# josegarciav/PINNs-RL-PDE

Measured on AMD Instinct MI355X. Metric: collocation-points/sec (residual+grad) + final residual L2, Burgers 1D, higher is better.
Workload: dtype f32

## Files before the change

include/pinn_jet.h:

```cpp
#ifndef PINN_JET_H
#define PINN_JET_H

#include <stddef.h>
#include <stdint.h>

#ifdef __cplusplus
extern "C" {
#endif

#define PINN_ABI_VERSION 2
#define PINN_MAX_LINEAR 24
#define PINN_MAX_STREAMS 7

#define PINN_FLAG_LAYER_NORM 1
#define PINN_FLAG_DETERMINISTIC 2
#define PINN_FLAG_LAYER_MAJOR 4
#define PINN_FLAG_WIDE_TILE32 8
#define PINN_FLAG_PLAIN_STREAMS 16
#define PINN_FLAG_SPACE_AXIS(a) ((a) << 8)
#define PINN_FLAG_SPACE_AXIS_MASK 0x300
#define PINN_FLAG_SPACE_DIRECTION(d0, d1, d2) \
  (((((d0) < 0 ? 2 : (d0)) & 3) << 10) | ((((d1) < 0 ? 2 : (d1)) & 3) << 12) | ((((d2) < 0 ? 2 : (d2)) & 3) << 14))
#define PINN_FLAG_SPACE_DIRECTION_MASK 0xFC00

typedef enum PinnStatus {
  PINN_OK = 0,
  PINN_ERR_BAD_DESC = -1,
  PINN_ERR_UNSUPPORTED = -2,
  PINN_ERR_MISALIGNED = -3,
  PINN_ERR_WORKSPACE = -4,
  PINN_ERR_HIP = -5,
  PINN_ERR_BAD_ORDER = -6
} PinnStatus;

typedef enum PinnArch {
  PINN_ARCH_FEEDFORWARD = 0,
  PINN_ARCH_FOURIER = 1,
  PINN_ARCH_SIREN = 2,
  PINN_ARCH_RESNET = 3,
  PINN_ARCH_ATTENTION = 4,
  PINN_ARCH_AUTOENCODER = 5
} PinnArch;

typedef enum PinnAct {
  PINN_ACT_TANH = 0,
  PINN_ACT_SIN = 1,
  PINN_ACT_GELU = 2,
  PINN_ACT_SIGMOID = 3,
  PINN_ACT_RELU = 4,
  PINN_ACT_LEAKY_RELU = 5,
  PINN_ACT_IDENTITY = 6
} PinnAct;

typedef enum PinnPde {
  PINN_PDE_BURGERS = 0,
  PINN_PDE_HEAT = 1,
  PINN_PDE_ALLEN_CAHN = 2,
  PINN_PDE_KDV = 3,
  PINN_PDE_CAHN_HILLIARD = 4,
  PINN_PDE_WAVE = 5,
  PINN_PDE_CONVECTION = 6,
  PINN_PDE_BLACK_SCHOLES = 7,
  PINN_PDE_PENDULUM = 8,
  PINN_PDE_HEAT_LAPLACIAN = 9
} PinnPde;

typedef enum PinnLoss { PINN_LOSS_MSE = 0, PINN_LOSS_MAE = 1, PINN_LOSS_HUBER = 2 } PinnLoss;

typedef struct PinnNetDesc {
  int32_t arch;
  int32_t activation;
  int32_t input_dim;
  int32_t num_linear;
  int32_t widths[PINN_MAX_LINEAR];
  int32_t mapping_size;
  float act_param;
  float ln_eps;
  int32_t num_blocks;
  int32_t flags;
} PinnNetDesc;

typedef struct PinnPdeDesc {
  int32_t kind;
  int32_t dimension;
  int32_t loss;
  float coef[4];
  float huber_delta;
} PinnPdeDesc;

int pinn_abi_version(void);
const char* pinn_last_error(void);

const char* pinn_build_info(void);

int pinn_num_tensors(const PinnNetDesc* net);

int pinn_pde_streams(const PinnPdeDesc* pde, int32_t* time_order, int32_t* space_order);

size_t pinn_workspace_bytes(const PinnNetDesc* net, int64_t N, int32_t time_order, int32_t space_order, int32_t backward);

typedef struct PinnKernelInfo {
  int32_t engine;
  int32_t time_order, space_order, act_family, backward;
  int32_t hmax, na0;
  int32_t grid;
  int32_t flush;
  int32_t default_mfma_form;
} PinnKernelInfo;
int pinn_kernel_for(const PinnNetDesc* net, int64_t N, int32_t time_order, int32_t space_order, int32_t backward,
                    PinnKernelInfo* out);
int pinn_kernel_name(const PinnNetDesc* net, int64_t N, int32_t time_order, int32_t space_order, int32_t backward,
                     char* buf, size_t len);

#define PINN_LM_MAX_PLAN 41
typedef struct PinnLmNodePlan {
  int32_t rows, depth;
  int32_t width;
  int32_t has_ln, has_skip, has_add;
  int32_t act_family;
  int32_t src_kind;
  int32_t fwd_fused;
  int32_t fwd_nch, fwd_rt, fwd_gy, fwd_aux;
  int32_t fwd_ew_kind;
  int32_t fwd_fpt;
  int32_t bwd_fused;
  int32_t bwd_nch, bwd_rt, bwd_gy, bwd_aux;
  int32_t bwd_ew_kind;
  int32_t bwd_fpt;
  int32_t head_fpt;
} PinnLmNodePlan;
int pinn_lm_plan(const PinnNetDesc* net, int64_t N, int32_t time_order, int32_t space_order, int32_t backward,
                 PinnLmNodePlan* out, int32_t max_records);

int pinn_unit_tail_plan(int64_t N, int32_t grid, int64_t* rounds, int32_t* groups, int64_t* first_tail_point);


int pinn_jet_forward(const PinnNetDesc* net, const float* const* weights, int32_t num_tensors, const float* x,
                     const float* t, int64_t N, int32_t time_order, int32_t space_order, float* const* jets_out,
                     void* workspace, size_t ws_bytes, void* stream);

int pinn_jet_backward(const PinnNetDesc* net, const float* const* weights, int32_t num_tensors, const float* x,
                      const float* t, int64_t N, int32_t time_order, int32_t space_order,
                      const float* const* jet_cotangents, float* const* weight_grads, void* workspace, size_t ws_bytes,
                      void* stream);

int pinn_jet_backward_inputs(const PinnNetDesc* net, const float* const* weights, int32_t num_tensors, const float* x,
                             const float* t, int64_t N, int32_t time_order, int32_t space_order,
                             const float* const* jet_cotangents, float* const* weight_grads,
                             float* x_grad, float* t_grad, void* workspace, size_t ws_bytes, void* stream);

int pinn_residual_forward(const PinnNetDesc* net, const float* const* weights, int32_t num_tensors,
                          const PinnPdeDesc* pde, const float* x, const float* t, int64_t N, float* residual_out,
                          float* loss_sum_out, void* workspace, size_t ws_bytes, void* stream);

int pinn_residual_loss_grad(const PinnNetDesc* net, const float* const* weights, int32_t num_tensors,
                            const PinnPdeDesc* pde, const float* x, const float* t, int64_t N, float grad_scale,
                            float* residual_out, float* loss_sum_out, float* const* weight_grads, void* workspace,
                            size_t ws_bytes, void* stream);

int pinn_residual_loss_grad_coef(const PinnNetDesc* net, const float* const* weights, int32_t num_tensors,
                                 const PinnPdeDesc* pde, const float* x, const float* t, int64_t N, float grad_scale,
                                 float* residual_out, float* loss_sum_out, float* const* weight_grads, float* coef_grads,
                                 void* workspace, size_t ws_bytes, void* stream);

int pinn_residual_loss_grad_inverse(const PinnNetDesc* net, const float* const* weights, int32_t num_tensors,
                                    const PinnPdeDesc* pde, const float* coef_values, const float* x, const float* t,
                                    int64_t N, float grad_scale, float* residual_out, float* loss_sum_out,
                                    float* const* weight_grads, float* coef_grads, void* workspace, size_t ws_bytes,
                                    void* stream);
size_t pinn_inverse_workspace_bytes(const PinnNetDesc* net, const PinnPdeDesc* pde, int64_t N);
int pinn_inverse_kernel_name(const PinnNetDesc* net, const PinnPdeDesc* pde, int64_t N, char* buf, size_t len);

int pinn_residual_backward(const PinnNetDesc* net, const float* const* weights, int32_t num_tensors,
                           const PinnPdeDesc* pde, const float* x, const float* t, int64_t N,
                           const float* residual_cotangent, float* const* weight_grads, void* workspace,
                           size_t ws_bytes, void* stream);

#define PINN_MAX_POINT_TERMS 8

int pinn_point_losses(const float* u, int32_t n_total, int32_t n_terms, const int32_t* lo, const int32_t* hi,
                      const float* const* targets, const float* weights, int32_t loss, float huber_delta,
                      float* term_losses, float* cotangent, const float* residual_sum, float residual_scale,
                      float residual_weight, int32_t n_boundary_terms, float* summary4, void* stream);

int pinn_jet_losses(const float* jets, int32_t n_streams, int32_t n_total, int32_t n_terms, const int32_t* lo, const int32_t* hi,
                    const int32_t* stream_of, const int32_t* pair_offset, const float* const* targets, const float* weights,
                    int32_t loss, float huber_delta, float* term_losses, float* cotangent, const float* residual_sum,
                    float residual_scale, float residual_weight, int32_t n_boundary_terms, float* summary4, void* stream);

#define PINN_FD_SCRATCH_DOUBLES 128
int pinn_fd_stencil_points(const float* x, const float* t, int64_t N, double eps, double x_lo, double x_hi, float* x3, float* t3,
                           void* stream);
int pinn_fd_smoothness(const float* u3, int64_t N, double eps, float weight, float* loss_out, float* cotangent3, float* summary4,
                       double* scratch, void* stream);

#define PINN_CAUSAL_MAX_BINS 64
#define PINN_CAUSAL_SCRATCH_DOUBLES (64 * 2 * PINN_CAUSAL_MAX_BINS)
int pinn_causal_weights(const float* residual, const float* t, int64_t N, int32_t n_bins, double t_lo, double t_hi,
                        const float* eps_dev, int32_t loss, float huber_delta, float grad_scale, float* cotangent,
                        float* loss_sum_out, float* plain_sum_out, float* bin_losses, float* bin_weights, double* scratch,
                        void* stream);

#define PINN_TERM_MAX_TERMS 16
#define PINN_TERM_MAX_FACTORS 4
#define PINN_TERM_SCRATCH_DOUBLES (64 * (1 + PINN_TERM_MAX_TERMS))

typedef enum PinnTermFactor {
  PINN_TERM_U = 0,
  PINN_TERM_UT = 1,
  PINN_TERM_UTT = 2,
  PINN_TERM_UX = 3,
  PINN_TERM_UXX = 4,
  PINN_TERM_UXXX = 5,
  PINN_TERM_UXXXX = 6,
  PINN_TERM_X = 7,
  PINN_TERM_T = 8,
  PINN_TERM_SIN_U = 9,
  PINN_TERM_COS_U = 10
} PinnTermFactor;

typedef struct PinnTermPdeTerm {
  int32_t n_factors;
  int32_t factor[PINN_TERM_MAX_FACTORS];
} PinnTermPdeTerm;

typedef struct PinnTermPde {
  int32_t time_order, space_order;
  int32_t n_terms;
  int32_t loss;
  float huber_delta;
  PinnTermPdeTerm terms[PINN_TERM_MAX_TERMS];
} PinnTermPde;

int pinn_term_residual(const PinnTermPde* pde, const float* coef_values, const float* jets, const float* x, const float* t,
                       int64_t N, float grad_scale, const float* residual_cotangent, float* residual_out, float* loss_sum_out,
                       float* jet_cotangents, float* coef_grads, double* scratch, void* stream);

#define PINN_TERM_UY 11
#define PINN_TERM_UYY 12
#define PINN_TERM_UZ 13
#define PINN_TERM_UZZ 14
#define PINN_TERM_Y 15
#define PINN_TERM_Z 16

typedef struct PinnTermPdeAxes {
  int32_t dimension;
  int32_t time_order;
  int32_t space_order[3];
  int32_t n_terms;
  int32_t loss;
  float huber_delta;
  PinnTermPdeTerm terms[PINN_TERM_MAX_TERMS];
} PinnTermPdeAxes;

int pinn_term_residual_axes(const PinnTermPdeAxes* pde, const float* coef_values, const float* const* jets, const float* x,
                            const float* t, int64_t N, float grad_scale, const float* residual_cotangent, float* residual_out,
                            float* loss_sum_out, float* const* jet_cotangents, float* coef_grads, double* scratch, void* stream);

#define PINN_TERM_UYYY 17
#define PINN_TERM_UYYYY 18
#define PINN_TERM_UZZZ 19
#define PINN_TERM_UZZZZ 20
#define PINN_TERM_UXY 21
#define PINN_TERM_UXZ 22
#define PINN_TERM_UYZ 23
#define PINN_TERM_UXXYY 24
#define PINN_TERM_UXXZZ 25
#define PINN_TERM_UYYZZ 26
#define PINN_TERM_MIXED_BLOCKS 9

typedef struct PinnTermPdeMixed {
  int32_t dimension;
  int32_t time_order;
  int32_t space_order[3];
  int32_t pair_order[3];
  int32_t n_terms;
  int32_t loss;
  float huber_delta;
  PinnTermPdeTerm terms[PINN_TERM_MAX_TERMS];
} PinnTermPdeMixed;

int pinn_term_residual_mixed(const PinnTermPdeMixed* pde, const float* coef_values, const float* const* jets, const float* x,
                             const float* t, int64_t N, float grad_scale, const float* residual_cotangent, float* residual_out,
                             float* loss_sum_out, float* const* jet_cotangents, float* coef_grads, double* scratch, void* stream);

#define PINN_SYSTEM_MAX_FIELDS 4
#define PINN_SYSTEM_MAX_EQUATIONS 4
#define PINN_SYSTEM_MAX_TERMS 32
#define PINN_SYSTEM_SCRATCH_DOUBLES (64 * (4 + 32))
#define PINN_SYSTEM_FACTOR(field, code) ((field) * 32 + (code))

typedef struct PinnTermPdeSystem {
  int32_t dimension;
  int32_t n_fields;
  int32_t n_equations;
  int32_t time_order[PINN_SYSTEM_MAX_FIELDS];
  int32_t space_order[PINN_SYSTEM_MAX_FIELDS][3];
  int32_t n_terms;
  int32_t equation_of[PINN_SYSTEM_MAX_TERMS];
  float eq_weight[PINN_SYSTEM_MAX_EQUATIONS];
  int32_t loss;
  float huber_delta;
  PinnTermPdeTerm terms[PINN_SYSTEM_MAX_TERMS];
} PinnTermPdeSystem;

int pinn_term_residual_system(const PinnTermPdeSystem* pde, const float* coef_values, const float* const* jets, const float* x,
                              const float* t, int64_t N, float grad_scale, const float* residual_cotangent, float* residual_out,
                              float* loss_sum_out, float* eq_loss_sums, float* const* jet_cotangents, float* coef_grads,
                              double* scratch, void* stream);

int pinn_adam_clip_step(float* params, const float* grads, float* exp_avg, float* exp_avg_sq, int64_t n, const float* lr,
                        float beta1, float beta2, float eps, float weight_decay, float max_norm, float* step,
                        float* scratch64, float* grad_norm_out, void* stream);

#define PINN_ADAPTIVE_RBW 0
#define PINN_ADAPTIVE_LRW 1
#define PINN_ADAPTIVE_SCRATCH_FLOATS 1296
int pinn_adaptive_adam_step(float* params, const float* comp_grads, int64_t ld, int32_t n_components,
                            const float* const* comp_losses, const float* loss_scales, int32_t strategy, double alpha,
                            double aw_eps, const float* initial_weights, float* state16, float* weights4_out, float* summary4,
                            float* exp_avg, float* exp_avg_sq, int64_t n, const float* lr, float beta1, float beta2, float eps,
                            float weight_decay, float max_norm, float* step, float* scratch, float* grad_norm_out,
                            float* grad_out, void* stream);

#define PINN_LBFGS_MAX_HISTORY 64
#define PINN_LBFGS_RECORD_DOUBLES 72
#define PINN_LBFGS_REC_LOSS 0
#define PINN_LBFGS_REC_GTD 1
#define PINN_LBFGS_REC_GMAX 2
#define PINN_LBFGS_REC_GSUM 3
#define PINN_LBFGS_REC_ACCEPTED 4
#define PINN_LBFGS_REC_COUNT 5
#define PINN_LBFGS_REC_ITER 6
#define PINN_LBFGS_REC_HDIAG 7
#define PINN_LBFGS_REC_DMAX 8
size_t pinn_lbfgs_state_bytes(int32_t history_size);
size_t pinn_lbfgs_scratch_bytes(int32_t history_size);
int pinn_lbfgs_direction(const float* grad, float* prev_grad, float* direction, float* ring, int64_t ld, int64_t n,
                         int32_t history_size, double t_prev, double* state, double* scratch, double* record, void* stream);
int pinn_lbfgs_eval_stats(const float* grad, const float* direction, int64_t n, const float* loss, double* scratch,
                          double* record, void* stream);

#ifdef __cplusplus
}
#endif
#endif
```

pinns-rl-pde_amd/_lib.py:

```python

from __future__ import annotations

import ctypes
import os
import subprocess
import threading

_HERE = os.path.dirname(os.path.abspath(__file__))
LIB_PATH = os.environ.get("PINN_LIB") or os.path.join(_HERE, "libpinnjet.so")
CSRC = os.path.join(_HERE, "csrc")

PINN_ABI_VERSION = 2
PINN_MAX_LINEAR = 24
PINN_MAX_STREAMS = 7
PINN_FLAG_LAYER_NORM = 1
PINN_FLAG_DETERMINISTIC = 2
PINN_FLAG_LAYER_MAJOR = 4
PINN_FLAG_WIDE_TILE32 = 8
PINN_FLAG_PLAIN_STREAMS = 16
PINN_FLAG_SPACE_AXIS_MASK = 0x300


def PINN_FLAG_SPACE_AXIS(axis: int) -> int:
    return (int(axis) << 8) & PINN_FLAG_SPACE_AXIS_MASK


PINN_FLAG_SPACE_DIRECTION_MASK = 0xFC00


def PINN_FLAG_SPACE_DIRECTION(d0: int = 0, d1: int = 0, d2: int = 0) -> int:
    bits = 0
    for a, d in enumerate((d0, d1, d2)):
        if d not in (-1, 0, 1):
            raise ValueError(f"direction entry {d!r}: -1, 0 or +1")
        bits |= (2 if d < 0 else int(d)) << (10 + 2 * a)
    return bits


ARCH = {"feedforward": 0, "fourier": 1, "siren": 2, "resnet": 3, "attention": 4, "autoencoder": 5}
ACT = {"tanh": 0, "sin": 1, "gelu": 2, "sigmoid": 3, "relu": 4, "leaky_relu": 5, "identity": 6}
PDE = {
    "burgers": 0, "heat": 1, "allen_cahn": 2, "kdv": 3, "cahn_hilliard": 4, "wave": 5, "convection": 6,
    "black_scholes": 7, "pendulum": 8, "heat_laplacian": 9,
}
LOSS = {"mse": 0, "mae": 1, "huber": 2}
ADAPTIVE = {"rbw": 0, "lrw": 1}
PINN_ADAPTIVE_SCRATCH_FLOATS = 1296
PINN_FD_SCRATCH_DOUBLES = 128
PINN_LBFGS_MAX_HISTORY = 64
PINN_LBFGS_RECORD_DOUBLES = 72
PINN_TERM_MAX_TERMS = 16
PINN_TERM_MAX_FACTORS = 4
PINN_TERM_SCRATCH_DOUBLES = 64 * (1 + PINN_TERM_MAX_TERMS)
PINN_CAUSAL_MAX_BINS = 64
PINN_CAUSAL_SCRATCH_DOUBLES = 64 * 2 * PINN_CAUSAL_MAX_BINS
TERM_FACTOR = {"u": 0, "u_t": 1, "u_tt": 2, "u_x": 3, "u_xx": 4, "u_xxx": 5, "u_xxxx": 6, "x": 7, "t": 8, "sin(u)": 9, "cos(u)": 10}
TERM_FACTOR_ND = dict(TERM_FACTOR, **{"u_y": 11, "u_yy": 12, "u_z": 13, "u_zz": 14, "y": 15, "z": 16})
TERM_FACTOR_MIXED = dict(TERM_FACTOR_ND, **{"u_yyy": 17, "u_yyyy": 18, "u_zzz": 19, "u_zzzz": 20, "u_xy": 21, "u_xz": 22, "u_yz": 23,
                                            "u_xxyy": 24, "u_xxzz": 25, "u_yyzz": 26})
PINN_TERM_MIXED_BLOCKS = 9
PINN_SYSTEM_MAX_FIELDS = 4
PINN_SYSTEM_MAX_EQUATIONS = 4
PINN_SYSTEM_MAX_TERMS = 32
PINN_SYSTEM_SCRATCH_DOUBLES = 64 * (4 + 32)


def PINN_SYSTEM_FACTOR(field: int, code: int) -> int:
    return int(field) * 32 + int(code)


LBFGS_REC = {"loss": 0, "gtd": 1, "gmax": 2, "gsum": 3, "accepted": 4, "count": 5, "n_iter": 6, "h_diag": 7, "dmax": 8}

EXPORTS = (
    "pinn_abi_version", "pinn_last_error", "pinn_build_info", "pinn_num_tensors", "pinn_pde_streams",
    "pinn_workspace_bytes", "pinn_jet_forward", "pinn_jet_backward", "pinn_residual_forward", "pinn_residual_backward",
    "pinn_residual_loss_grad", "pinn_residual_loss_grad_coef", "pinn_point_losses", "pinn_jet_losses", "pinn_adam_clip_step",
    "pinn_jet_backward_inputs", "pinn_kernel_for", "pinn_kernel_name", "pinn_residual_loss_grad_inverse",
    "pinn_inverse_workspace_bytes", "pinn_inverse_kernel_name", "pinn_adaptive_adam_step", "pinn_lbfgs_state_bytes",
    "pinn_lbfgs_scratch_bytes", "pinn_lbfgs_direction", "pinn_lbfgs_eval_stats", "pinn_fd_stencil_points", "pinn_fd_smoothness",
    "pinn_unit_tail_plan", "pinn_term_residual", "pinn_causal_weights", "pinn_term_residual_axes",
    "pinn_term_residual_mixed", "pinn_lm_plan", "pinn_term_residual_system",
)


class PinnNetDesc(ctypes.Structure):
    _fields_ = [
        ("arch", ctypes.c_int32), ("activation", ctypes.c_int32), ("input_dim", ctypes.c_int32),
        ("num_linear", ctypes.c_int32), ("widths", ctypes.c_int32 * PINN_MAX_LINEAR),
        ("mapping_size", ctypes.c_int32), ("act_param", ctypes.c_float), ("ln_eps", ctypes.c_float),
        ("num_blocks", ctypes.c_int32), ("flags", ctypes.c_int32),
    ]


class PinnPdeDesc(ctypes.Structure):
    _fields_ = [
        ("kind", ctypes.c_int32), ("dimension", ctypes.c_int32), ("loss", ctypes.c_int32),
        ("coef", ctypes.c_float * 4), ("huber_delta", ctypes.c_float),
    ]


class PinnTermPdeTerm(ctypes.Structure):
    _fields_ = [("n_factors", ctypes.c_int32), ("factor", ctypes.c_int32 * PINN_TERM_MAX_FACTORS)]


class PinnTermPde(ctypes.Structure):
    _fields_ = [
        ("time_order", ctypes.c_int32), ("space_order", ctypes.c_int32), ("n_terms", ctypes.c_int32), ("loss", ctypes.c_int32),
        ("huber_delta", ctypes.c_float), ("terms", PinnTermPdeTerm * PINN_TERM_MAX_TERMS),
    ]


class PinnTermPdeAxes(ctypes.Structure):
    _fields_ = [
        ("dimension", ctypes.c_int32), ("time_order", ctypes.c_int32), ("space_order", ctypes.c_int32 * 3),
        ("n_terms", ctypes.c_int32), ("loss", ctypes.c_int32), ("huber_delta", ctypes.c_float),
        ("terms", PinnTermPdeTerm * PINN_TERM_MAX_TERMS),
    ]


class PinnTermPdeMixed(ctypes.Structure):
    _fields_ = [
        ("dimension", ctypes.c_int32), ("time_order", ctypes.c_int32), ("space_order", ctypes.c_int32 * 3),
        ("pair_order", ctypes.c_int32 * 3), ("n_terms", ctypes.c_int32), ("loss", ctypes.c_int32),
        ("huber_delta", ctypes.c_float), ("terms", PinnTermPdeTerm * PINN_TERM_MAX_TERMS),
    ]


class PinnTermPdeSystem(ctypes.Structure):
    _fields_ = [
        ("dimension", ctypes.c_int32), ("n_fields", ctypes.c_int32), ("n_equations", ctypes.c_int32),
        ("time_order", ctypes.c_int32 * PINN_SYSTEM_MAX_FIELDS), ("space_order", (ctypes.c_int32 * 3) * PINN_SYSTEM_MAX_FIELDS),
        ("n_terms", ctypes.c_int32), ("equation_of", ctypes.c_int32 * PINN_SYSTEM_MAX_TERMS),
        ("eq_weight", ctypes.c_float * PINN_SYSTEM_MAX_EQUATIONS), ("loss", ctypes.c_int32), ("huber_delta", ctypes.c_float),
        ("terms", PinnTermPdeTerm * PINN_SYSTEM_MAX_TERMS),
    ]


class PinnKernelInfo(ctypes.Structure):
    _fields_ = [
        ("engine", ctypes.c_int32), ("time_order", ctypes.c_int32), ("space_order", ctypes.c_int32),
        ("act_family", ctypes.c_int32), ("backward", ctypes.c_int32), ("hmax", ctypes.c_int32), ("na0", ctypes.c_int32),
        ("grid", ctypes.c_int32), ("flush", ctypes.c_int32), ("default_mfma_form", ctypes.c_int32),
    ]


PINN_LM_MAX_PLAN = 41


class PinnLmNodePlan(ctypes.Structure):
    _fields_ = [(f, ctypes.c_int32) for f in (
        "rows", "depth", "width", "has_ln", "has_skip", "has_add", "act_family", "src_kind",
        "fwd_fused", "fwd_nch", "fwd_rt", "fwd_gy", "fwd_aux", "fwd_ew_kind", "fwd_fpt",
        "bwd_fused", "bwd_nch", "bwd_rt", "bwd_gy", "bwd_aux", "bwd_ew_kind", "bwd_fpt", "head_fpt")]


ENGINE_LAYER_MAJOR, ENGINE_TILE_MAJOR = 0, 1
FLUSH = {0: "direct", 1: "store", 2: "two_level", 3: "deterministic"}


class JetLibraryError(RuntimeError):
    """The HIP library is missing, stale, or returned an error code."""


_lib = None
_lock = threading.Lock()


def build(verbose: bool = False) -> str:
    cmd = ["make", "-C", CSRC, "-j", str(min(8, os.cpu_count() or 1))]
    res = subprocess.run(cmd, stdout=subprocess.PIPE, stderr=subprocess.STDOUT, text=True)
    if verbose or res.returncode:
        print(res.stdout)
    if res.returncode:
        raise JetLibraryError(f"building libpinnjet.so failed (exit {res.returncode})")
    return LIB_PATH


def load():
    global _lib
    if _lib is not None:
        return _lib
    with _lock:
        if _lib is not None:
            return _lib
        if not os.path.exists(LIB_PATH):
            raise JetLibraryError(
                f"{LIB_PATH} not found: the HIP extension is not built (run `python -c 'import __graft_entry__ as g; "
                "g.build()'` or `make -C pinns-rl-pde_amd/csrc`).  There is no CPU fallback."
            )
        import torch

        lib = ctypes.CDLL(LIB_PATH)
        vp, i32, i64, f32 = ctypes.c_void_p, ctypes.c_int32, ctypes.c_int64, ctypes.c_float
        P = ctypes.POINTER
        lib.pinn_abi_version.restype = ctypes.c_int
        lib.pinn_abi_version.argtypes = []
        lib.pinn_last_error.restype = ctypes.c_char_p
        lib.pinn_last_error.argtypes = []
        lib.pinn_build_info.restype = ctypes.c_char_p
        lib.pinn_build_info.argtypes = []
        lib.pinn_num_tensors.restype = ctypes.c_int
        lib.pinn_num_tensors.argtypes = [P(PinnNetDesc)]
        lib.pinn_pde_streams.restype = ctypes.c_int
        lib.pinn_pde_streams.argtypes = [P(PinnPdeDesc), P(i32), P(i32)]
        lib.pinn_workspace_bytes.restype = ctypes.c_size_t
        lib.pinn_workspace_bytes.argtypes = [P(PinnNetDesc), i64, i32, i32, i32]
        sz = ctypes.c_size_t
        lib.pinn_kernel_for.restype = ctypes.c_int
        lib.pinn_kernel_for.argtypes = [P(PinnNetDesc), i64, i32, i32, i32, P(PinnKernelInfo)]
        lib.pinn_kernel_name.restype = ctypes.c_int
        lib.pinn_kernel_name.argtypes = [P(PinnNetDesc), i64, i32, i32, i32, ctypes.c_char_p, sz]
        lib.pinn_lm_plan.restype = ctypes.c_int
        lib.pinn_lm_plan.argtypes = [P(PinnNetDesc), i64, i32, i32, i32, P(PinnLmNodePlan), i32]
        lib.pinn_jet_forward.restype = ctypes.c_int
        lib.pinn_jet_forward.argtypes = [P(PinnNetDesc), P(vp), i32, vp, vp, i64, i32, i32, P(vp), vp, sz, vp]
        lib.pinn_jet_backward.restype = ctypes.c_int
        lib.pinn_jet_backward.argtypes = [P(PinnNetDesc), P(vp), i32, vp, vp, i64, i32, i32, P(vp), P(vp), vp, sz, vp]
        lib.pinn_jet_backward_inputs.restype = ctypes.c_int
        lib.pinn_jet_backward_inputs.argtypes = [P(PinnNetDesc), P(vp), i32, vp, vp, i64, i32, i32, P(vp), P(vp), vp, vp, vp,
                                                 sz, vp]
        lib.pinn_residual_forward.restype = ctypes.c_int
        lib.pinn_residual_forward.argtypes = [P(PinnNetDesc), P(vp), i32, P(PinnPdeDesc), vp, vp, i64, vp, vp, vp, sz, vp]
        lib.pinn_residual_backward.restype = ctypes.c_int
        lib.pinn_residual_backward.argtypes = [P(PinnNetDesc), P(vp), i32, P(PinnPdeDesc), vp, vp, i64, vp, P(vp), vp, sz,
                                               vp]
        lib.pinn_residual_loss_grad.restype = ctypes.c_int
        lib.pinn_residual_loss_grad.argtypes = [P(PinnNetDesc), P(vp), i32, P(PinnPdeDesc), vp, vp, i64, f32, vp, vp,
                                                P(vp), vp, sz, vp]
        lib.pinn_residual_loss_grad_coef.restype = ctypes.c_int
        lib.pinn_residual_loss_grad_coef.argtypes = [P(PinnNetDesc), P(vp), i32, P(PinnPdeDesc), vp, vp, i64, f32, vp, vp,
                                                     P(vp), vp, vp, sz, vp]
        lib.pinn_residual_loss_grad_inverse.restype = ctypes.c_int
        lib.pinn_residual_loss_grad_inverse.argtypes = [P(PinnNetDesc), P(vp), i32, P(PinnPdeDesc), vp, vp, vp, i64, f32, vp, vp,
                                                        P(vp), vp, vp, sz, vp]
        lib.pinn_inverse_workspace_bytes.restype = ctypes.c_size_t
        lib.pinn_inverse_workspace_bytes.argtypes = [P(PinnNetDesc), P(PinnPdeDesc), i64]
        lib.pinn_inverse_kernel_name.restype = ctypes.c_int
        lib.pinn_inverse_kernel_name.argtypes = [P(PinnNetDesc), P(PinnPdeDesc), i64, ctypes.c_char_p, sz]
        lib.pinn_point_losses.restype = ctypes.c_int
        lib.pinn_point_losses.argtypes = [vp, i32, i32, P(i32), P(i32), P(vp), P(f32), i32, f32, vp, vp, vp, f32, f32, i32, vp, vp]
        lib.pinn_jet_losses.restype = ctypes.c_int
        lib.pinn_jet_losses.argtypes = [vp, i32, i32, i32, P(i32), P(i32), P(i32), P(i32), P(vp), P(f32), i32, f32, vp, vp, vp, f32, f32,
                                        i32, vp, vp]
        lib.pinn_adam_clip_step.restype = ctypes.c_int
        lib.pinn_adam_clip_step.argtypes = [vp, vp, vp, vp, i64, vp, f32, f32, f32, f32, f32, vp, vp, vp, vp]
        f64 = ctypes.c_double
        lib.pinn_adaptive_adam_step.restype = ctypes.c_int
        lib.pinn_adaptive_adam_step.argtypes = [vp, vp, i64, i32, P(vp), P(f32), i32, f64, f64, P(f32), vp, vp, vp, vp, vp, i64, vp,
                                                f32, f32, f32, f32, f32, vp, vp, vp, vp, vp]
        lib.pinn_lbfgs_state_bytes.restype = ctypes.c_size_t
        lib.pinn_lbfgs_state_bytes.argtypes = [i32]
        lib.pinn_lbfgs_scratch_bytes.restype = ctypes.c_size_t
        lib.pinn_lbfgs_scratch_bytes.argtypes = [i32]
        lib.pinn_lbfgs_direction.restype = ctypes.c_int
        lib.pinn_lbfgs_direction.argtypes = [vp, vp, vp, vp, i64, i64, i32, f64, vp, vp, vp, vp]
        lib.pinn_lbfgs_eval_stats.restype = ctypes.c_int
        lib.pinn_lbfgs_eval_stats.argtypes = [vp, vp, i64, vp, vp, vp, vp]
        lib.pinn_fd_stencil_points.restype = ctypes.c_int
        lib.pinn_fd_stencil_points.argtypes = [vp, vp, i64, f64, f64, f64, vp, vp, vp]
        lib.pinn_fd_smoothness.restype = ctypes.c_int
        lib.pinn_fd_smoothness.argtypes = [vp, i64, f64, f32, vp, vp, vp, vp, vp]
        lib.pinn_unit_tail_plan.restype = ctypes.c_int
        lib.pinn_unit_tail_plan.argtypes = [i64, i32, P(i64), P(i32), P(i64)]
        lib.pinn_term_residual.restype = ctypes.c_int
        lib.pinn_term_residual.argtypes = [P(PinnTermPde), vp, vp, vp, vp, i64, f32, vp, vp, vp, vp, vp, vp, vp]
        lib.pinn_term_residual_axes.restype = ctypes.c_int
        lib.pinn_term_residual_axes.argtypes = [P(PinnTermPdeAxes), vp, P(vp), vp, vp, i64, f32, vp, vp, vp, P(vp), vp, vp, vp]
        lib.pinn_term_residual_mixed.restype = ctypes.c_int
        lib.pinn_term_residual_mixed.argtypes = [P(PinnTermPdeMixed), vp, P(vp), vp, vp, i64, f32, vp, vp, vp, P(vp), vp, vp, vp]
        lib.pinn_term_residual_system.restype = ctypes.c_int
        lib.pinn_term_residual_system.argtypes = [P(PinnTermPdeSystem), vp, P(vp), vp, vp, i64, f32, vp, vp, vp, vp, P(vp), vp, vp, vp]
        lib.pinn_causal_weights.restype = ctypes.c_int
        lib.pinn_causal_weights.argtypes = [vp, vp, i64, i32, f64, f64, vp, i32, f32, f32, vp, vp, vp, vp, vp, vp, vp]
        if lib.pinn_abi_version() != PINN_ABI_VERSION:
            raise JetLibraryError(f"libpinnjet.so ABI {lib.pinn_abi_version()} != expected {PINN_ABI_VERSION}: rebuild")
        _lib = lib
    return _lib


def build_info() -> str:
    return load().pinn_build_info().decode("utf-8", "replace")


def kernel_for(prog, N: int, nt: int, nx: int, backward: int) -> dict:
    info = PinnKernelInfo()
    check(load().pinn_kernel_for(ctypes.byref(prog.desc), int(N), int(nt), int(nx), int(backward), ctypes.byref(info)))
    out = {f: getattr(info, f) for f, _ in PinnKernelInfo._fields_}
    out["engine"] = "tile_major" if info.engine == ENGINE_TILE_MAJOR else "layer_major"
    out["flush"] = FLUSH.get(info.flush)
    out["default_mfma_form"] = bool(info.default_mfma_form)
    return out


def lm_plan(prog, N: int, nt: int, nx: int, backward: int) -> list:
    recs = (PinnLmNodePlan * PINN_LM_MAX_PLAN)()
    n = load().pinn_lm_plan(ctypes.byref(prog.desc), int(N), int(nt), int(nx), int(backward), recs, PINN_LM_MAX_PLAN)
    if n < 0:
        check(n)
    return [{f: getattr(recs[m], f) for f, _ in PinnLmNodePlan._fields_} for m in range(n + 1)]


def kernel_name(prog, N: int, nt: int, nx: int, backward: int) -> str:
    buf = ctypes.create_string_buffer(64)
    check(load().pinn_kernel_name(ctypes.byref(prog.desc), int(N), int(nt), int(nx), int(backward), buf, len(buf)))
    return buf.value.decode("ascii")


def u16_tail_plan(N: int, grid: int) -> tuple:
    r, g, f = ctypes.c_int64(), ctypes.c_int32(), ctypes.c_int64()
    check(load().pinn_unit_tail_plan(int(N), int(grid), ctypes.byref(r), ctypes.byref(g), ctypes.byref(f)))
    return r.value, g.value, f.value


def check(rc: int) -> None:
    if rc != 0:
        msg = load().pinn_last_error().decode("utf-8", "replace")
        if rc == -6:
            raise ValueError(msg)
        if rc == -2:
            raise NotImplementedError(f"pinn_jet: {msg}")
        raise JetLibraryError(f"pinn_jet error {rc}: {msg}")
```

pinns-rl-pde_amd/csrc/jet_kernel_u16.h:

```cpp
#pragma once
#include "jet_kernel_wide.h"

namespace pinn {

#define U16_BARRIER(idx)     \
  do {                       \
    PINN_STAMP(idx);         \
    __syncthreads();         \
    PINN_STAMP(ST_BARRIER);  \
  } while (0)

constexpr int kU = 16;
constexpr int kUP = 132;
constexpr int kUThreads = 512;
constexpr int kUWaves = 8;
constexpr int kUH = 128;
constexpr int kUImgS = kU * kUP;

__device__ __forceinline__ f32x4 mfma16(float a, float b, f32x4 c) {
  return __builtin_amdgcn_mfma_f32_16x16x4f32(a, b, c, 0, 0, 0);
}

__device__ __forceinline__ int u16_opaque(int v) {
  asm volatile("" : "+v"(v));
  return v;
}

template <int NT, int NX>
__device__ __forceinline__ void u16_enc_preact(const float* ep, int din, const float* xin, int j, int n, float* z) {
  constexpr int K = 1 + NT + NX;
#pragma unroll
  for (int s = 0; s < K; ++s) z[s] = 0.0f;
  float v = ep[kMaxDin * kUH + j];
  float wt = 0.0f;
#pragma unroll
  for (int c = 0; c < kMaxDin; ++c) {
    const float w = ep[c * kUH + j];
    v = fmaf(xin[c * kU + n], w, v);
    wt = c == din - 1 ? w : wt;
  }
  z[0] = v;
  if constexpr (NT >= 1) z[1] = wt;
  if constexpr (NX >= 1) z[1 + NT] = ep[j];
}

template <int ACT, int NT, int NX, bool MRG = false>
__device__ __forceinline__ void u16_encode(const NetDev& net, const float* ep, const float* xin, float* dst, int tid, float cc = 0.0f) {
  constexpr int K = 1 + NT + NX;
  const int n = tid & 15;
  const int din = net.din;
  float* row = dst + n * kUP;
  if (net.enc == ENC_FOURIER) {
    const int M = net.enc_out >> 1;
#pragma unroll 1
    for (int m = tid >> 4; m < M; m += kUThreads / kU) {
      float z[K], ys[K], yc[K];
      u16_enc_preact<NT, NX>(ep, din, xin, m, n, z);
      float sn, cs;
      fast_sincosf(z[0], &sn, &cs);
      const float fs[6] = {sn, cs, -sn, -cs, sn, cs};
      const float fc[6] = {cs, -sn, -cs, sn, cs, -sn};
      ys[0] = sn;
      yc[0] = cs;
      if constexpr (MRG) {
        merged_fwd(fs, cc, z, ys);
        merged_fwd(fc, cc, z, yc);
      } else {
        dir_fwd<NT>(fs, z + 1, ys + 1);
        dir_fwd<NX>(fs, z + 1 + NT, ys + 1 + NT);
        dir_fwd<NT>(fc, z + 1, yc + 1);
        dir_fwd<NX>(fc, z + 1 + NT, yc + 1 + NT);
      }
#pragma unroll
      for (int s = 0; s < K; ++s) {
        row[s * kUImgS + m] = ys[s];
        row[s * kUImgS + M + m] = yc[s];
      }
    }
  } else {
    const int H = net.enc_out;
#pragma unroll 1
    for (int f = tid >> 4; f < H; f += kUThreads / kU) {
      float z[K], y[K];
      u16_enc_preact<NT, NX>(ep, din, xin, f, n, z);
      if constexpr (MRG) act_fwd_merged<ACT>(net.enc_param, cc, z, y);
      else act_fwd<ACT, NT, NX>(net.enc_param, z, y);
#pragma unroll
      for (int s = 0; s < K; ++s) row[s * kUImgS + f] = y[s];
    }
  }
}

__device__ __forceinline__ unsigned u16_rows_off(int row0, int ld, int c, int g) {
  return static_cast<unsigned>((row0 + c) * ld + 4 * g) * 4u;
}
__device__ __forceinline__ unsigned u16_cols_off(int col0, int ld, int c, int g) {
  return static_cast<unsigned>(4 * g * ld + col0 + c) * 4u;
}
template <bool COLS>
__device__ __forceinline__ f32x4 u16_wload(const float* W, int ld, unsigned off, int b) {
  if constexpr (COLS) {
    f32x4 v;
#pragma unroll
    for (int m = 0; m < 4; ++m) v[m] = *reinterpret_cast<const float*>(reinterpret_cast<const char*>(W + (long long)(16 * b + m) * ld) + off);
    return v;
  } else {
    return *reinterpret_cast<const f32x4*>(reinterpret_cast<const char*>(W + 16 * b) + off);
  }
}

template <int K, int NB, bool COLS>
__device__ __forceinline__ void u16_gemm_n(f32x4 (&acc)[K], const float* W, int ld, unsigned off, f32x4 w0, f32x4 w1, const float* xl) {
  f32x4 wq[3];
  wq[0] = w0;
  wq[1] = w1;
  f32x4 bc[K], bn[K];
#pragma unroll
  for (int s = 0; s < K; ++s) bc[s] = *reinterpret_cast<const f32x4*>(xl + s * kUImgS);
#pragma unroll
  for (int b = 0; b < NB; ++b) {
    if (b + 2 < NB) wq[(b + 2) % 3] = u16_wload<COLS>(W, ld, off, b + 2);
    if (b + 1 < NB) {
#pragma unroll
      for (int s = 0; s < K; ++s) bn[s] = *reinterpret_cast<const f32x4*>(xl + s * kUImgS + 16 * (b + 1));
    }
    __builtin_amdgcn_sched_barrier(0);
#pragma unroll
    for (int m = 0; m < 4; ++m)
#pragma unroll
      for (int s = 0; s < K; ++s) acc[s] = mfma16(wq[b % 3][m], bc[s][m], acc[s]);
    __builtin_amdgcn_sched_barrier(0);
    if (b + 1 < NB) {
#pragma unroll
      for (int s = 0; s < K; ++s) bc[s] = bn[s];
    }
  }
}

template <int K, bool COLS>
__device__ __forceinline__ void u16_gemm(f32x4 (&acc)[K], const float* W, int ld, unsigned off, f32x4 w0, f32x4 w1, int nb, const float* xl) {
  switch (nb) {
    case 8: u16_gemm_n<K, 8, COLS>(acc, W, ld, off, w0, w1, xl); return;
    case 4: u16_gemm_n<K, 4, COLS>(acc, W, ld, off, w0, w1, xl); return;
    default: break;
  }
#pragma unroll 1
  for (int b = 0; b < nb; ++b) {
    const f32x4 w = b == 0 ? w0 : b == 1 ? w1 : u16_wload<COLS>(W, ld, off, b);
#pragma unroll
    for (int m = 0; m < 4; ++m)
#pragma unroll
      for (int s = 0; s < K; ++s) acc[s] = mfma16(w[m], xl[s * kUImgS + 16 * b + m], acc[s]);
  }
}

template <int K, int NA, int OFF, int NPT>
__device__ __forceinline__ void u16_outer_n(f32x4 (&pt)[NPT], const float* zl, const float* al) {
  float zc, zn, ac[NA], an[NA];
  zc = zl[0];
#pragma unroll
  for (int t = 0; t < NA; ++t) ac[t] = al[16 * t];
#pragma unroll
  for (int st = 0; st < 4 * K; ++st) {
    if (st + 1 < 4 * K) {
      const int s = (st + 1) >> 2, m = (st + 1) & 3;
      zn = zl[s * kUImgS + m * kUP];
#pragma unroll
      for (int t = 0; t < NA; ++t) an[t] = al[s * kUImgS + m * kUP + 16 * t];
    }
    __builtin_amdgcn_sched_barrier(0);
#pragma unroll
    for (int t = 0; t < NA; ++t) pt[OFF + t] = mfma16(zc, ac[t], pt[OFF + t]);
    __builtin_amdgcn_sched_barrier(0);
    if (st + 1 < 4 * K) {
      zc = zn;
#pragma unroll
      for (int t = 0; t < NA; ++t) ac[t] = an[t];
    }
  }
}

template <int K, int OFF, int NMAX, int NPT>
__device__ __forceinline__ void u16_outer(f32x4 (&pt)[NPT], int na, const float* zl, const float* al) {
  if constexpr (NMAX >= 8) {
    if (na * 2 == NMAX) { u16_outer_n<K, NMAX / 2, OFF, NPT>(pt, zl, al); return; }
  }
  u16_outer_n<K, NMAX, OFF, NPT>(pt, zl, al);
}

#ifndef PINN_U16_PACK
#define PINN_U16_PACK 1
#endif
constexpr int kUPackMax = 3;

template <int NB, bool COLS>
__device__ __forceinline__ void u16p_gemm_n(f32x4 (&acc)[kUPackMax], int G, const float* W, int ld, unsigned off, f32x4 w0, f32x4 w1, const float* xl) {
  f32x4 wq[3];
  wq[0] = w0;
  wq[1] = w1;
  f32x4 bc[kUPackMax], bn[kUPackMax];
#pragma unroll
  for (int j = 0; j < kUPackMax; ++j) {
    bc[j] = f32x4{0.0f, 0.0f, 0.0f, 0.0f};
    bn[j] = bc[j];
    if (j < G) bc[j] = *reinterpret_cast<const f32x4*>(xl + 4 * j * kUP);
  }
#pragma unroll
  for (int b = 0; b < NB; ++b) {
    if (b + 2 < NB) wq[(b + 2) % 3] = u16_wload<COLS>(W, ld, off, b + 2);
    if (b + 1 < NB) {
#pragma unroll
      for (int j = 0; j < kUPackMax; ++j)
        if (j < G) bn[j] = *reinterpret_cast<const f32x4*>(xl + 4 * j * kUP + 16 * (b + 1));
    }
#pragma unroll
    for (int j = 0; j < kUPackMax; ++j) {
      if (j < G) {
#pragma unroll
        for (int m = 0; m < 4; ++m) acc[j] = mfma16(wq[b % 3][m], bc[j][m], acc[j]);
      }
    }
    if (b + 1 < NB) {
#pragma unroll
      for (int j = 0; j < kUPackMax; ++j) bc[j] = bn[j];
    }
  }
}

template <bool COLS>
__device__ __forceinline__ void u16p_gemm(f32x4 (&acc)[kUPackMax], int G, const float* W, int ld, unsigned off, f32x4 w0, f32x4 w1, int nb, const float* xl) {
  switch (nb) {
    case 8: u16p_gemm_n<8, COLS>(acc, G, W, ld, off, w0, w1, xl); return;
    case 4: u16p_gemm_n<4, COLS>(acc, G, W, ld, off, w0, w1, xl); return;
    default: break;
  }
#pragma unroll 1
  for (int b = 0; b < nb; ++b) {
    const f32x4 w = b == 0 ? w0 : b == 1 ? w1 : u16_wload<COLS>(W, ld, off, b);
#pragma unroll
    for (int j = 0; j < kUPackMax; ++j) {
      if (j < G) {
#pragma unroll
        for (int m = 0; m < 4; ++m) acc[j] = mfma16(w[m], xl[4 * j * kUP + 16 * b + m], acc[j]);
      }
    }
  }
}

template <int K, int NA, int OFF, int NPT>
__device__ __forceinline__ void u16p_outer_n(f32x4 (&pt)[NPT], int G, const float* zl, const float* al) {
#pragma unroll
  for (int j = 0; j < kUPackMax; ++j) {
    if (j < G) {
      float zc, zn = 0.0f, ac[NA], an[NA];
      zc = zl[4 * j * kUP];
#pragma unroll
      for (int t = 0; t < NA; ++t) {
        ac[t] = al[4 * j * kUP + 16 * t];
        an[t] = 0.0f;
      }
#pragma unroll
      for (int s = 0; s < K; ++s) {
        if (s + 1 < K) {
          zn = zl[(s + 1) * kUImgS + 4 * j * kUP];
#pragma unroll
          for (int t = 0; t < NA; ++t) an[t] = al[(s + 1) * kUImgS + 4 * j * kUP + 16 * t];
        }
        __builtin_amdgcn_sched_barrier(0);
#pragma unroll
        for (int t = 0; t < NA; ++t) pt[OFF + t] = mfma16(zc, ac[t], pt[OFF + t]);
        __builtin_amdgcn_sched_barrier(0);
        if (s + 1 < K) {
          zc = zn;
#pragma unroll
          for (int t = 0; t < NA; ++t) ac[t] = an[t];
        }
      }
    }
  }
}

template <int K, int OFF, int NMAX, int NPT>
__device__ __forceinline__ void u16p_outer(f32x4 (&pt)[NPT], int G, int na, const float* zl, const float* al) {
  if constexpr (NMAX >= 8) {
    if (na * 2 == NMAX) { u16p_outer_n<K, NMAX / 2, OFF, NPT>(pt, G, zl, al); return; }
  }
  u16p_outer_n<K, NMAX, OFF, NPT>(pt, G, zl, al);
}

__device__ __forceinline__ void u16_wave_sync() {
  __builtin_amdgcn_fence(__ATOMIC_RELEASE, "wavefront");
  __builtin_amdgcn_wave_barrier();
  __builtin_amdgcn_fence(__ATOMIC_ACQUIRE, "wavefront");
}

template <int ACT, int NT, int NX, bool MRG = false>
__device__ __forceinline__ void u16_ew_forward(f32x4 (&v)[1 + NT + NX], float w, f32x4 (&rec)[1 + NT + NX], float cc = 0.0f) {
  constexpr int K = 1 + NT + NX;
#pragma unroll
  for (int r = 0; r < 4; ++r) {
    float z[K], y[K];
#pragma unroll
    for (int s = 0; s < K; ++s) z[s] = v[s][r];
    if constexpr (MRG) act_fwd_merged<ACT>(w, cc, z, y);
    else act_fwd<ACT, NT, NX>(w, z, y);
    rec[0][r] = ActTape<ACT>::value_is_output ? y[0] : z[0];
#pragma unroll
    for (int s = 1; s < K; ++s) rec[s][r] = z[s];
#pragma unroll
    for (int s = 0; s < K; ++s) v[s][r] = y[s];
  }
}

template <int K>
__device__ __forceinline__ void u16_put(float* il, const f32x4 (&v)[K]) {
#pragma unroll
  for (int s = 0; s < K; ++s) *reinterpret_cast<f32x4*>(il + s * kUImgS) = v[s];
}
template <int K>
__device__ __forceinline__ void u16_get(const float* il, f32x4 (&v)[K]) {
#pragma unroll
  for (int s = 0; s < K; ++s) v[s] = *reinterpret_cast<const f32x4*>(il + s * kUImgS);
}

template <int ACT, int NT, int NX, bool MRG = false>
__device__ __forceinline__ float u16_ew_backward(f32x4 (&ab)[1 + NT + NX], float w, const f32x4 (&rec)[1 + NT + NX], float cc = 0.0f) {
  constexpr int K = 1 + NT + NX;
  float part = 0.0f;
#pragma unroll
  for (int r = 0; r < 4; ++r) {
    float z[K], abv[K], zb[K];
#pragma unroll
    for (int s = 0; s < K; ++s) {
      z[s] = rec[s][r];
      abv[s] = ab[s][r];
    }
    if constexpr (MRG) part += act_bwd_tape_merged<ACT>(w, cc, z, abv, zb);
    else act_bwd_tape<ACT, NT, NX>(w, z, abv, zb);
#pragma unroll
    for (int s = 0; s < K; ++s) ab[s][r] = zb[s];
  }
  return part;
}

template <int ACT, int NT, int NX, bool MRG>
__device__ __forceinline__ void u16_act_replay(float w, float cc, const float* z, float* y) {
  if constexpr (MRG) act_fwd_tape_merged<ACT>(w, cc, z, y);
  else act_fwd_tape<ACT, NT, NX>(w, z, y);
}

__device__ __forceinline__ f32x4 row16_sum4(f32x4 v) {
#pragma unroll
  for (int r = 0; r < 4; ++r) v[r] = row16_sum(v[r]);
  return v;
}

template <int ACT, int NT, int NX, bool BWD, int NA0, bool COEF = false, bool MRG = false>
__global__ __launch_bounds__(kUThreads, 1) void jet_kernel_u16(const KernelArgs a) {
  static_assert(!MRG || (NT == 1 && NX == 1), "the merged set is laid out as the (1,1) set");
  constexpr int K = 1 + NT + NX;
  constexpr int NKT = kUH / 16;
  constexpr int NPT = NA0 + (kPersist - 1) * NKT;
  static_assert(kPersist == 3, "the layer -> tile-offset table below is written for three persistent layers");
  constexpr int img = K * kUImgS;
  extern __shared__ __attribute__((aligned(16))) float smem[];
  const NetDev& net = a.net;
  float* X = smem;
  float* A2 = X + img;
  float* REC = A2 + img;
  constexpr bool KEEP = MRG && BWD;
  [[maybe_unused]] float* S = REC + 2 * img;
  float* UP = REC + (KEEP ? 3 : 2) * img;
  float* xin2 = UP + kUWaves * K * kU;
  float* wb = xin2 + 2 * kMaxDin * kU;
  float* ep = wb + (1 + kPersist) * kUH;
  float* pl = ep + (kMaxDin + 1) * kUH;
  float* pdwl = pl + (kPersist + kMaxDin + 1) * kUH;
  float* psl = pdwl + 4 * kUThreads;
  float* xint = psl + 2 * kU;
  [[maybe_unused]] float* pcl = xint + kMaxDin * kU;
  auto mcoef = [&]() -> float {
    if constexpr (MRG) return -X[kUH + 2];
    else return 0.0f;
  };
  auto cadd = [&](float part, bool own) {
    if constexpr (MRG && COEF) {
      if (own) pcl[u16_opaque(threadIdx.x)] += part;
    }
  };

  PINN_STAMP_DECL
  const int tid = threadIdx.x;
  const int wv = __builtin_amdgcn_readfirstlane(tid >> 6);
  const int lane = tid & 63;
  const int g = lane >> 4, c = lane & 15;
  const int din = net.din;
  const int nl = net.n_layers;
#if PINN_U16_PACK
  const long long NL = a.u16_loop_points;
#else
  const long long NL = a.N;
#endif
  const long long nunits = (NL + kU - 1) / kU;
  const int frow = 16 * wv + 4 * g;
  const int ioff = c * kUP + frow;

  for (int k = tid; k < kUH; k += kUThreads) {
    wb[k] = k < net.h_last ? net.w_out[k] : 0.0f;
    for (int l = 0; l < nl; ++l) wb[(1 + l) * kUH + k] = k < net.layer[l].out_dim ? net.layer[l].b[k] : 0.0f;
  }
  stage_enc_params<kUH>(net, ep, tid);
#pragma unroll
  for (int i = 0; i < kPersist + kMaxDin + 1; ++i)
    if (tid < kUH) pl[i * kUH + tid] = 0.0f;
  const float b_out0 = net.b_out[0];
  static_assert(!COEF || BWD, "coefficient cotangents belong to the reverse launch");
  if constexpr (COEF) {
    if (tid < kU) {
      X[tid * kUP + kUH] = 0.0f;
      X[tid * kUP + kUH + 1] = 0.0f;
    }
  }
  if (tid < 4) {
    const float cv = tid == 0 ? a.pde.c0 : tid == 1 ? a.pde.c1 : tid == 2 ? a.pde.c2 : a.pde.c3;
    X[tid * kUP + kUH + 2] = COEF ? a.pde.coef_dev[tid] : cv;
  }

  f32x4 pt[NPT];
#pragma unroll
  for (int t = 0; t < NPT; ++t) pt[t] = f32x4{0.0f, 0.0f, 0.0f, 0.0f};
  if constexpr (BWD) *reinterpret_cast<f32x4*>(pdwl + 4 * tid) = f32x4{0.0f, 0.0f, 0.0f, 0.0f};
  if (tid < 2 * kU) psl[tid] = 0.0f;
  if constexpr (MRG && COEF) pcl[tid] = 0.0f;

  float xr[kMaxDin] = {0.0f, 0.0f, 0.0f, 0.0f};
  [[maybe_unused]] float xv = 0.0f;
  static_assert(kMaxDin * kU == 64, "the merged units' coordinate lanes are wave 0");
  auto mfetch = [&](long long p, bool ok) {
    const int cc = u16_opaque(tid) >> 4;
    const bool live = ok && cc < din;
    const bool space = live && cc < din - 1;
    unsigned long long bx = reinterpret_cast<unsigned long long>(a.x), bt = reinterpret_cast<unsigned long long>(a.t);
    asm volatile("" : "+s"(bx), "+s"(bt));
    const long long idx = p * (space ? din - 1 : live ? 1 : 0) + (space ? cc : 0);
    using gfloat = const float __attribute__((address_space(1)));
    xv = *(gfloat*)(bt + (space ? bx - bt : 0ull) + 4ull * static_cast<unsigned long long>(idx));
  };
  auto mput = [&](float* dst, bool ok) {
    const int to = u16_opaque(tid);
    dst[to] = ok && (to >> 4) < din ? xv : 0.0f;
  };
  auto unit_point = [&](long long u, bool& ok) -> long long {
    const long long p = u * kU + (u16_opaque(tid) & 15);
    ok = u < nunits && p < NL;
    return p;
  };
  auto at_point = [&](long long p0, int npts, bool& ok) -> long long {
    const int n = u16_opaque(tid) & 15;
    ok = n < npts && p0 + n < a.N;
    return p0 + n;
  };
  auto fetch_coords = [&](long long u) {
    if constexpr (MRG) {
      if (wv == 0) {
        bool ok;
        const long long p = unit_point(u, ok);
        mfetch(p, ok);
      }
    } else if (tid < kU) {
      const long long p = u * kU + tid;
      const bool ok = u < nunits && p < NL;
#pragma unroll
      for (int cc = 0; cc < kMaxDin; ++cc) {
        if (cc < din - 1) xr[cc] = ok ? a.x[p * (din - 1) + cc] : 0.0f;
        if (cc == din - 1) xr[cc] = ok ? a.t[p] : 0.0f;
      }
    }
  };
  auto fetch_coords_at = [&](long long p0, int npts) {
    if constexpr (MRG) {
      if (wv == 0) {
        bool ok;
        const long long p = at_point(p0, npts, ok);
        mfetch(p, ok);
      }
    } else if (tid < kU) {
      const long long p = p0 + tid;
      const bool ok = tid < npts && p < a.N;
#pragma unroll
      for (int cc = 0; cc < kMaxDin; ++cc) {
        if (cc < din - 1) xr[cc] = ok ? a.x[p * (din - 1) + cc] : 0.0f;
        if (cc == din - 1) xr[cc] = ok ? a.t[p] : 0.0f;
      }
    }
  };
  auto put_xr = [&](float* dst) {
    if (tid < kU) {
#pragma unroll
      for (int cc = 0; cc < kMaxDin; ++cc) dst[cc * kU + tid] = xr[cc];
    }
  };
  auto put_coords = [&](float* dst, [[maybe_unused]] long long us) {
    if constexpr (MRG) {
      if (wv == 0) {
        bool ok;
        unit_point(us, ok);
        mput(dst, ok);
      }
    } else {
      put_xr(dst);
    }
  };
  auto put_coords_at = [&](float* dst, [[maybe_unused]] long long p0, [[maybe_unused]] int npts) {
    if constexpr (MRG) {
      if (wv == 0) {
        bool ok;
        at_point(p0, npts, ok);
        mput(dst, ok);
      }
    } else {
      put_xr(dst);
    }
  };
#if PINN_U16_PACK
  if (a.u16_tail_groups > 0) {
    const long long tp0 = a.u16_loop_points + 4LL * a.u16_tail_groups * blockIdx.x;
    fetch_coords_at(tp0, 4 * a.u16_tail_groups);
    put_coords_at(xint, tp0, 4 * a.u16_tail_groups);
  }
#endif
  fetch_coords(blockIdx.x);
  put_coords(xin2, blockIdx.x);
  if constexpr (MRG) fetch_coords(blockIdx.x + gridDim.x);
  int xpar = 0;

  for (long long u = blockIdx.x; u < nunits; u += gridDim.x) {
    const long long p0 = u * kU;
    U16_BARRIER(ST_BWD_FLUSH);
    const float* xin = xin2 + xpar * (kMaxDin * kU);
    float* xin_next = xin2 + (xpar ^ 1) * (kMaxDin * kU);
    xpar ^= 1;
    if constexpr (!MRG) fetch_coords(u + gridDim.x);
    f32x4 w0, w1;
    {
      const LayerDev L0 = uniform_layer(net.layer[0]);
      const unsigned off = u16_rows_off(16 * wv < L0.out_dim ? 16 * wv : 0, L0.ld, c, g);
      w0 = u16_wload<false>(L0.W, L0.ld, off, 0);
      w1 = u16_wload<false>(L0.W, L0.ld, off, L0.in_dim > 16 ? 1 : 0);
    }
    PINN_STAMP(ST_STAGE);
    float* src = (MRG || (nl & 1)) ? X : A2;
    float* dst = (MRG || (nl & 1)) ? A2 : X;
    u16_encode<ACT, NT, NX, MRG>(net, ep, xin, src, u16_opaque(tid), mcoef());
    U16_BARRIER(ST_ENCODE);

    f32x4 acc[K];
    for (int l = 0; l < nl; ++l) {
      const LayerDev Ly = uniform_layer(net.layer[l]);
      const bool on = 16 * wv < Ly.out_dim;
      const bool last = l + 1 == nl;
#pragma unroll
      for (int s = 0; s < K; ++s) acc[s] = f32x4{0.0f, 0.0f, 0.0f, 0.0f};
      if (on) {
        u16_gemm<K, false>(acc, Ly.W, Ly.ld, u16_rows_off(16 * wv, Ly.ld, c, g), w0, w1, Ly.in_dim >> 4, src + c * kUP + 4 * g);
        acc[0] += *reinterpret_cast<const f32x4*>(wb + (1 + l) * kUH + frow);
      }
      if (l == 0) {
        put_coords(xin_next, u + gridDim.x);
      }
      if constexpr (MRG) {
        if (last) fetch_coords(u + 2 * gridDim.x);
      }
      PINN_STAMP(ST_FWD_GEMM);
      if (!last) {
        {
          const LayerDev Ln = uniform_layer(net.layer[l + 1]);
          const unsigned off = u16_rows_off(16 * wv < Ln.out_dim ? 16 * wv : 0, Ln.ld, c, g);
          w0 = u16_wload<false>(Ln.W, Ln.ld, off, 0);
          w1 = u16_wload<false>(Ln.W, Ln.ld, off, Ln.in_dim > 16 ? 1 : 0);
        }
        if (on) {
          f32x4 rec[K];
          u16_ew_forward<ACT, NT, NX, MRG>(acc, Ly.act_param, rec, mcoef());
          if constexpr (BWD) u16_put<K>(REC + l * img + ioff, rec);
        }
        if (on) u16_put<K>(dst + ioff, acc);
        U16_BARRIER(ST_FWD_EW);
        float* const t = src;
        src = dst;
        dst = t;
      } else if (on) {
        f32x4 rec[K];
        u16_ew_forward<ACT, NT, NX, MRG>(acc, Ly.act_param, rec, mcoef());
        if constexpr (BWD) u16_put<K>((KEEP ? S : A2) + ioff, rec);
      }
    }
    PINN_STAMP(ST_FWD_EW);

    {
      const f32x4 w4 = *reinterpret_cast<const f32x4*>(wb + frow);
      float po[K];
#pragma unroll
      for (int s = 0; s < K; ++s) {
        po[s] = fmaf(w4[0], acc[s][0], fmaf(w4[1], acc[s][1], fmaf(w4[2], acc[s][2], w4[3] * acc[s][3])));
        po[s] += __shfl_xor(po[s], 16);
        po[s] += __shfl_xor(po[s], 32);
      }
      if (g == 0) {
#pragma unroll
        for (int s = 0; s < K; ++s) UP[(wv * K + s) * kU + c] = po[s];
      }
    }
    U16_BARRIER(ST_OUT);

    float ub[K];
    {
      const long long p = p0 + c;
      const bool ok = p < NL;
      const bool writer = tid < kU;
      float j[K];
#pragma unroll
      for (int s = 0; s < K; ++s) {
        float v = s == 0 ? b_out0 : 0.0f;
#pragma unroll
        for (int w = 0; w < kUWaves; ++w) v += UP[(w * K + s) * kU + c];
        j[s] = v;
      }
      if (a.mode == MODE_JETS) {
#pragma unroll
        for (int s = 0; s < K; ++s) {
          if (writer && ok && a.jets_out[s]) a.jets_out[s][p] = j[s];
          ub[s] = (BWD && ok && a.jets_bar[s]) ? a.jets_bar[s][p] : 0.0f;
        }
      } else {
        float d[K];
        PdeDev pde = a.pde;
        pde.c0 = X[0 * kUP + kUH + 2];
        pde.c1 = X[1 * kUP + kUH + 2];
        pde.c2 = X[2 * kUP + kUH + 2];
        pde.c3 = X[3 * kUP + kUH + 2];
        float r;
        if constexpr (MRG) r = pde_residual_merged(j, d);
        else r = pde_residual<NT, NX>(pde, j, xin[c], d);
        float dl;
        float lt = loss_term(pde, r, &dl);
        if (!ok) {
          lt = 0.0f;
          dl = 0.0f;
        }
        if (writer && ok && a.residual_out) a.residual_out[p] = r;
        if (writer) psl[c] += lt;
        const float rb = !BWD ? 0.0f : a.res_bar ? (ok ? a.res_bar[p] : 0.0f) : a.grad_scale * dl;
#pragma unroll
        for (int s = 0; s < K; ++s) ub[s] = rb * d[s];
        if constexpr (COEF && !MRG) {
          float dc0, dc1;
          pde_coef_grads<NT, NX>(pde, j, xin[c], dc0, dc1);
          if (writer) {
            X[c * kUP + kUH] += rb * dc0;
            X[c * kUP + kUH + 1] += rb * dc1;
          }
        }
      }
    }

    PINN_STAMP(ST_EPI);
    if constexpr (!BWD) continue;
    if (tid < kU) psl[kU + c] += ub[0];
    f32x4 ab[K];
    {
      const LayerDev Lz = uniform_layer(net.layer[nl - 1]);
      const f32x4 w4 = *reinterpret_cast<const f32x4*>(wb + frow);
#pragma unroll
      for (int s = 0; s < K; ++s) ab[s] = w4 * ub[s];
      if (16 * wv < Lz.out_dim) {
        f32x4 rec[K];
        u16_get<K>((KEEP ? S : A2) + ioff, rec);
        float* const pdwp = pdwl + 4 * u16_opaque(tid);
        f32x4 pdw = *reinterpret_cast<const f32x4*>(pdwp);
#pragma unroll
        for (int r = 0; r < 4; ++r) {
          float z[K], y[K];
#pragma unroll
          for (int s = 0; s < K; ++s) z[s] = rec[s][r];
          if constexpr (KEEP) {
#pragma unroll
            for (int s = 0; s < K; ++s) y[s] = acc[s][r];
          } else {
            u16_act_replay<ACT, NT, NX, MRG>(Lz.act_param, mcoef(), z, y);
          }
          float gg = 0.0f;
#pragma unroll
          for (int s = 0; s < K; ++s) gg = fmaf(ub[s], y[s], gg);
          pdw[r] += gg;
        }
        *reinterpret_cast<f32x4*>(pdwp) = pdw;
        cadd(u16_ew_backward<ACT, NT, NX, MRG>(ab, Lz.act_param, rec, mcoef()), true);
        if constexpr (KEEP) u16_put<K>(S + ioff, ab);
      }
    }
    PINN_STAMP(ST_B0);

    for (int l = nl - 1; l >= 0; --l) {
      const LayerDev Ly = uniform_layer(net.layer[l]);
      const bool on = 16 * wv < Ly.out_dim;
      const bool need_abar = l > 0 || net.enc == ENC_LINEAR;
      const bool kon = 16 * wv < Ly.in_dim;
      if constexpr (!KEEP) {
        if (l + 1 < nl || nl == 1) U16_BARRIER(ST_BWD_EW);
        if (on) u16_put<K>(X + ioff, ab);
      }
      const float* const ZB = !KEEP ? X : l + 1 == nl ? S : REC + l * img;
      const float* const AP = !KEEP || (l & 1) ? A2 : X;
      float pw = 0.0f;
      if constexpr (KEEP) {
        if (l > 0) pw = uniform_layer(net.layer[l - 1]).act_param;
      } else if (l > 0) {
        const LayerDev P = uniform_layer(net.layer[l - 1]);
        pw = P.act_param;
        if (kon) {
          f32x4 rec[K], y[K];
          u16_get<K>(REC + (l - 1) * img + ioff, rec);
#pragma unroll
          for (int r = 0; r < 4; ++r) {
            float z[K], yy[K];
#pragma unroll
            for (int s = 0; s < K; ++s) z[s] = rec[s][r];
            u16_act_replay<ACT, NT, NX, MRG>(pw, mcoef(), z, yy);
#pragma unroll
            for (int s = 0; s < K; ++s) y[s][r] = yy[s];
          }
          u16_put<K>(A2 + ioff, y);
        }
      } else {
        u16_encode<ACT, NT, NX, MRG>(net, ep, xin, A2, u16_opaque(tid), mcoef());
      }
      const unsigned coff = u16_cols_off(kon ? 16 * wv : 0, Ly.ld, c, g);
      if (need_abar) {
        w0 = u16_wload<true>(Ly.W, Ly.ld, coff, 0);
        w1 = u16_wload<true>(Ly.W, Ly.ld, coff, 1);
      }
      U16_BARRIER(ST_BWD_PUT);
      if (Ly.db && tid < Ly.out_dim) {
        float gsum = 0.0f;
#pragma unroll
        for (int n = 0; n < kU; ++n) gsum += ZB[n * kUP + tid];
        pl[l * kUH + tid] += gsum;
      }
      PINN_STAMP(ST_BWD_DB);
      const bool dw_first = wv >= 4;
#pragma unroll
      for (int half = 0; half < 2; ++half) {
        if ((half == 0) == dw_first && on && Ly.dW) {
          const float* zl = ZB + 4 * g * kUP + 16 * wv + c;
          const float* al = AP + 4 * g * kUP + c;
          const int na = Ly.in_dim >> 4;
          if (l == 0) u16_outer<K, 0, NA0, NPT>(pt, na, zl, al);
          else if (l == 1) u16_outer<K, NA0, NKT, NPT>(pt, na, zl, al);
          else u16_outer<K, NA0 + NKT, NKT, NPT>(pt, na, zl, al);
        }
        if ((half == 0) == dw_first) PINN_STAMP(ST_BWD_STREAM);
        if (half == 1) break;
        if (need_abar) {
#pragma unroll
          for (int s = 0; s < K; ++s) ab[s] = f32x4{0.0f, 0.0f, 0.0f, 0.0f};
          if (kon) u16_gemm<K, true>(ab, Ly.W, Ly.ld, coff, w0, w1, Ly.out_dim >> 4, ZB + c * kUP + 4 * g);
        }
        PINN_STAMP(ST_BWD_DX);
        if (l > 0 && kon) {
          f32x4 rec[K];
          u16_get<K>(REC + (l - 1) * img + ioff, rec);
          cadd(u16_ew_backward<ACT, NT, NX, MRG>(ab, pw, rec, mcoef()), true);
          if constexpr (KEEP) u16_put<K>(REC + (l - 1) * img + ioff, ab);
        }
        PINN_STAMP(ST_BWD_EW);
      }
      if constexpr (KEEP) {
        if (l == 1 && nl > 2) {
          u16_encode<ACT, NT, NX, MRG>(net, ep, xin, X, u16_opaque(tid), mcoef());
          PINN_STAMP(ST_ENCODE);
        }
      }
      if constexpr (MRG && COEF) {
        if (l == 0 && net.enc == ENC_FOURIER && kon) {
          f32x4 aw[1] = {f32x4{0.0f, 0.0f, 0.0f, 0.0f}};
          {
            const float* xl = ZB + kUImgS + c * kUP + 4 * g;
            const int nb = Ly.out_dim >> 4;
#pragma unroll 1
            for (int b = 0; b < nb; ++b) {
              const f32x4 w = u16_wload<true>(Ly.W, Ly.ld, coff, b);
              const f32x4 xv = *reinterpret_cast<const f32x4*>(xl + 16 * b);
#pragma unroll
              for (int m = 0; m < 4; ++m) aw[0] = mfma16(w[m], xv[m], aw[0]);
            }
          }
          const int M = net.enc_out >> 1;
          const f32x4 val = *reinterpret_cast<const f32x4*>(AP + ioff);
          float part = 0.0f;
#pragma unroll
          for (int r = 0; r < 4; ++r) {
            const int jf = frow + r;
            part = fmaf(aw[0][r], fourier_coef_partial_merged(ep[jf < M ? jf : jf - M], val[r]), part);
          }
          cadd(part, true);
        }
      }
    }

    if (net.enc == ENC_LINEAR && (net.d_encW || (MRG && COEF))) {
      const int H = net.enc_out;
      const bool enc_sums = !(MRG && COEF) || net.d_encW != nullptr;
      U16_BARRIER(ST_ENC_BWD);
      if (16 * wv < H) {
#pragma unroll
        for (int r = 0; r < 4; ++r) {
          float z[K], abv[K], zb[K];
          u16_enc_preact<NT, NX>(ep, din, xin, frow + r, c, z);
#pragma unroll
          for (int s = 0; s < K; ++s) abv[s] = ab[s][r];
          if constexpr (MRG) cadd(act_bwd_merged<ACT>(net.enc_param, mcoef(), z, abv, zb), true);
          else act_bwd<ACT, NT, NX>(net.enc_param, z, abv, zb);
#pragma unroll
          for (int s = 0; s < K; ++s) ab[s][r] = zb[s];
        }
        if (enc_sums) u16_put<K>(X + ioff, ab);
      }
      U16_BARRIER(ST_ENC_BWD);
      const int te = u16_opaque(tid);
      if (enc_sums && te < H) {
        float gb = 0.0f, gt = 0.0f, gx = 0.0f;
        float gw[kMaxDin] = {0.0f, 0.0f, 0.0f, 0.0f};
#pragma unroll 4
        for (int n = 0; n < kU; ++n) {
          const float vv = X[n * kUP + te];
          gb += vv;
#pragma unroll
          for (int cc = 0; cc < kMaxDin; ++cc)
            if (cc < din) gw[cc] = fmaf(vv, xin[cc * kU + n], gw[cc]);
          if constexpr (NT >= 1) gt += X[1 * kUImgS + n * kUP + te];
          if constexpr (NX >= 1) gx += X[(1 + NT) * kUImgS + n * kUP + te];
        }
#pragma unroll
        for (int cc = 0; cc < kMaxDin; ++cc) pl[(kPersist + cc) * kUH + te] += gw[cc] + (cc == din - 1 ? gt : 0.0f) + (cc == 0 ? gx : 0.0f);
        pl[(kPersist + kMaxDin) * kUH + te] += gb;
      }
      PINN_STAMP(ST_ENC_BWD);
    }
  }

#if PINN_U16_PACK
  if (a.u16_tail_groups > 0) {
    const int G = a.u16_tail_groups;
    const int tp = u16_opaque(tid);
    const int gp = (tp & 63) >> 4, cp = tp & 15;
    const int sp = cp >> 2, qp = cp & 3;
    const int frowp = 16 * wv + 4 * gp;
    const int boff = (sp < K ? sp : 0) * kUImgS + qp * kUP + 4 * gp;
    const int woff = sp * kUImgS + qp * kUP + frowp;
    const int eoff = qp * kUP + frowp;
    const bool wcol = sp < K;
    const bool writer = tp < 4;
    const long long tail_p0 = a.u16_loop_points + 4LL * G * blockIdx.x;
    auto acc_put = [&](float* im, const f32x4 (&pa)[kUPackMax]) {
#pragma unroll
      for (int j = 0; j < kUPackMax; ++j)
        if (j < G && wcol) *reinterpret_cast<f32x4*>(im + woff + 4 * j * kUP) = pa[j];
      u16_wave_sync();
    };

    U16_BARRIER(ST_BWD_FLUSH);
    const float* xin = xint;
    f32x4 w0, w1;
    {
      const LayerDev L0 = uniform_layer(net.layer[0]);
      const unsigned off = u16_rows_off(16 * wv < L0.out_dim ? 16 * wv : 0, L0.ld, cp, gp);
      w0 = u16_wload<false>(L0.W, L0.ld, off, 0);
      w1 = u16_wload<false>(L0.W, L0.ld, off, L0.in_dim > 16 ? 1 : 0);
    }
    PINN_STAMP(ST_STAGE);
    float* src = (nl & 1) ? X : A2;
    float* dst = (nl & 1) ? A2 : X;
    u16_encode<ACT, NT, NX, MRG>(net, ep, xin, src, tp, mcoef());
    U16_BARRIER(ST_ENCODE);

    for (int l = 0; l < nl; ++l) {
      const LayerDev Ly = uniform_layer(net.layer[l]);
      const bool on = 16 * wv < Ly.out_dim;
      const bool last = l + 1 == nl;
      f32x4 pa[kUPackMax];
#pragma unroll
      for (int j = 0; j < kUPackMax; ++j) pa[j] = f32x4{0.0f, 0.0f, 0.0f, 0.0f};
      if (on) u16p_gemm<false>(pa, G, Ly.W, Ly.ld, u16_rows_off(16 * wv, Ly.ld, cp, gp), w0, w1, Ly.in_dim >> 4, src + boff);
      PINN_STAMP(ST_FWD_GEMM);
      if (!last) {
        const LayerDev Ln = uniform_layer(net.layer[l + 1]);
        const unsigned off = u16_rows_off(16 * wv < Ln.out_dim ? 16 * wv : 0, Ln.ld, cp, gp);
        w0 = u16_wload<false>(Ln.W, Ln.ld, off, 0);
        w1 = u16_wload<false>(Ln.W, Ln.ld, off, Ln.in_dim > 16 ? 1 : 0);
      }
      if (on) acc_put(dst, pa);
      const f32x4 bias = *reinterpret_cast<const f32x4*>(wb + (1 + l) * kUH + frowp);
      const f32x4 w4 = *reinterpret_cast<const f32x4*>(wb + frowp);
#pragma unroll
      for (int j = 0; j < kUPackMax; ++j) {
        if (j < G) {
          f32x4 v[K];
#pragma unroll
          for (int s = 0; s < K; ++s) v[s] = f32x4{0.0f, 0.0f, 0.0f, 0.0f};
          if (!last) {
            if (on) {
              u16_get<K>(dst + eoff + 4 * j * kUP, v);
              v[0] += bias;
              f32x4 rec[K];
              u16_ew_forward<ACT, NT, NX, MRG>(v, Ly.act_param, rec, mcoef());
              if constexpr (BWD) u16_put<K>(REC + l * img + eoff + 4 * j * kUP, rec);
              u16_put<K>(dst + eoff + 4 * j * kUP, v);
            }
          } else if (on) {
            u16_get<K>(dst + eoff + 4 * j * kUP, v);
            v[0] += bias;
            f32x4 rec[K];
            u16_ew_forward<ACT, NT, NX, MRG>(v, Ly.act_param, rec, mcoef());
            if constexpr (BWD) u16_put<K>(A2 + eoff + 4 * j * kUP, rec);
          }
          if (last) {
            float po[K];
#pragma unroll
            for (int s = 0; s < K; ++s) {
              po[s] = fmaf(w4[0], v[s][0], fmaf(w4[1], v[s][1], fmaf(w4[2], v[s][2], w4[3] * v[s][3])));
              po[s] += __shfl_xor(po[s], 16);
              po[s] += __shfl_xor(po[s], 32);
            }
            if (gp == 0 && sp == 0) {
#pragma unroll
              for (int s = 0; s < K; ++s) UP[(wv * K + s) * kU + 4 * j + qp] = po[s];
            }
          }
        }
      }
      if (!last) {
        U16_BARRIER(ST_FWD_EW);
        float* const t = src;
        src = dst;
        dst = t;
      }
    }
    U16_BARRIER(ST_OUT);

    [[maybe_unused]] const float* park = A2;
#pragma unroll 1
    for (int jg = 0; jg < G; ++jg) {
      float ub[K];
      const int pp = 4 * jg + qp;
      {
        const long long p = tail_p0 + pp;
        const bool ok = p < a.N;
        float j[K];
#pragma unroll
        for (int s = 0; s < K; ++s) {
          float v = s == 0 ? b_out0 : 0.0f;
#pragma unroll
          for (int w = 0; w < kUWaves; ++w) v += UP[(w * K + s) * kU + pp];
          j[s] = v;
        }
        if (a.mode == MODE_JETS) {
#pragma unroll
          for (int s = 0; s < K; ++s) {
            if (writer && ok && a.jets_out[s]) a.jets_out[s][p] = j[s];
            ub[s] = (BWD && ok && a.jets_bar[s]) ? a.jets_bar[s][p] : 0.0f;
          }
        } else {
          float d[K];
          PdeDev pde = a.pde;
          pde.c0 = X[0 * kUP + kUH + 2];
          pde.c1 = X[1 * kUP + kUH + 2];
          pde.c2 = X[2 * kUP + kUH + 2];
          pde.c3 = X[3 * kUP + kUH + 2];
          float r;
          if constexpr (MRG) r = pde_residual_merged(j, d);
          else r = pde_residual<NT, NX>(pde, j, xin[pp], d);
          float dl;
          float lt = loss_term(pde, r, &dl);
          if (!ok) {
            lt = 0.0f;
            dl = 0.0f;
          }
          if (writer && ok && a.residual_out) a.residual_out[p] = r;
          if (writer) psl[pp] += lt;
          const float rb = !BWD ? 0.0f : a.res_bar ? (ok ? a.res_bar[p] : 0.0f) : a.grad_scale * dl;
#pragma unroll
          for (int s = 0; s < K; ++s) ub[s] = rb * d[s];
          if constexpr (COEF && !MRG) {
            float dc0, dc1;
            pde_coef_grads<NT, NX>(pde, j, xin[pp], dc0, dc1);
            if (writer) {
              X[pp * kUP + kUH] += rb * dc0;
              X[pp * kUP + kUH + 1] += rb * dc1;
            }
          }
        }
      }
      PINN_STAMP(ST_EPI);
      if constexpr (!BWD) continue;
      if (writer) psl[kU + pp] += ub[0];
      f32x4 ab[K];
      {
        const LayerDev Lz = uniform_layer(net.layer[nl - 1]);
        const f32x4 w4 = *reinterpret_cast<const f32x4*>(wb + frowp);
#pragma unroll
        for (int s = 0; s < K; ++s) ab[s] = w4 * ub[s];
        if (16 * wv < Lz.out_dim) {
          f32x4 rec[K];
          float* const rp = A2 + eoff + 4 * jg * kUP;
          u16_get<K>(rp, rec);
          if (sp == 0) {
            float* const pdwp = pdwl + 4 * tp;
            f32x4 pdw = *reinterpret_cast<const f32x4*>(pdwp);
#pragma unroll
            for (int r = 0; r < 4; ++r) {
              float z[K], y[K];
#pragma unroll
              for (int s = 0; s < K; ++s) z[s] = rec[s][r];
              u16_act_replay<ACT, NT, NX, MRG>(Lz.act_param, mcoef(), z, y);
              float gg = 0.0f;
#pragma unroll
              for (int s = 0; s < K; ++s) gg = fmaf(ub[s], y[s], gg);
              pdw[r] += gg;
            }
            *reinterpret_cast<f32x4*>(pdwp) = pdw;
          }
          cadd(u16_ew_backward<ACT, NT, NX, MRG>(ab, Lz.act_param, rec, mcoef()), sp == 0);
          u16_put<K>(rp, ab);
        }
      }
      PINN_STAMP(ST_B0);
    }

    if constexpr (BWD) {
      for (int l = nl - 1; l >= 0; --l) {
        const LayerDev Ly = uniform_layer(net.layer[l]);
        const bool on = 16 * wv < Ly.out_dim;
        const bool need_abar = l > 0 || net.enc == ENC_LINEAR;
        const bool kon = 16 * wv < Ly.in_dim;
        auto unpark = [&]() {
#pragma unroll
          for (int j = 0; j < kUPackMax; ++j) {
            if (j < G && on) {
              f32x4 zb[K];
              u16_get<K>(park + eoff + 4 * j * kUP, zb);
              u16_put<K>(X + eoff + 4 * j * kUP, zb);
            }
          }
        };
        const bool top = l + 1 == nl;
        if (top) unpark();
        if (!top || nl == 1) U16_BARRIER(ST_BWD_EW);
        if (!top) unpark();
        float pw = 0.0f;
        u16_wave_sync();
        if (l > 0) {
          const LayerDev P = uniform_layer(net.layer[l - 1]);
          pw = P.act_param;
          if (kon) {
#pragma unroll
            for (int j = 0; j < kUPackMax; ++j) {
              if (j < G) {
                f32x4 rec[K], y[K];
                u16_get<K>(REC + (l - 1) * img + eoff + 4 * j * kUP, rec);
#pragma unroll
                for (int r = 0; r < 4; ++r) {
                  float z[K], yy[K];
#pragma unroll
                  for (int s = 0; s < K; ++s) z[s] = rec[s][r];
                  u16_act_replay<ACT, NT, NX, MRG>(pw, mcoef(), z, yy);
#pragma unroll
                  for (int s = 0; s < K; ++s) y[s][r] = yy[s];
                }
                u16_put<K>(A2 + eoff + 4 * j * kUP, y);
              }
            }
          }
        } else {
          u16_encode<ACT, NT, NX, MRG>(net, ep, xin, A2, tp, mcoef());
        }
        const unsigned coff = u16_cols_off(kon ? 16 * wv : 0, Ly.ld, cp, gp);
        if (need_abar) {
          w0 = u16_wload<true>(Ly.W, Ly.ld, coff, 0);
          w1 = u16_wload<true>(Ly.W, Ly.ld, coff, 1);
        }
        U16_BARRIER(ST_BWD_PUT);
        if (Ly.db && tp < Ly.out_dim) {
          float gsum = 0.0f;
          for (int n = 0; n < 4 * G; ++n) gsum += X[n * kUP + tp];
          pl[l * kUH + tp] += gsum;
        }
        PINN_STAMP(ST_BWD_DB);
        if (need_abar) {
          f32x4 pa[kUPackMax];
#pragma unroll
          for (int j = 0; j < kUPackMax; ++j) pa[j] = f32x4{0.0f, 0.0f, 0.0f, 0.0f};
          if (kon) u16p_gemm<true>(pa, G, Ly.W, Ly.ld, coff, w0, w1, Ly.out_dim >> 4, X + boff);
          PINN_STAMP(ST_BWD_DX);
          float* const xch = REC + (l > 0 ? l - 1 : 0) * img;
#pragma unroll
          for (int j = 0; j < kUPackMax; ++j) {
            if (j < G) {
              f32x4 rec[K];
              if (l > 0) {
                if (kon) u16_get<K>(xch + eoff + 4 * j * kUP, rec);
                u16_wave_sync();
              }
              if (kon && wcol) *reinterpret_cast<f32x4*>(xch + woff + 4 * j * kUP) = pa[j];
              if (l > 0) {
                u16_wave_sync();
                if (kon) {
                  f32x4 ab[K];
                  u16_get<K>(xch + eoff + 4 * j * kUP, ab);
                  cadd(u16_ew_backward<ACT, NT, NX, MRG>(ab, pw, rec, mcoef()), sp == 0);
                  u16_put<K>(xch + eoff + 4 * j * kUP, ab);
                }
              }
            }
          }
          park = xch;
          PINN_STAMP(ST_BWD_EW);
        }
        if (on && Ly.dW) {
          const float* zl = X + gp * kUP + 16 * wv + cp;
          const float* al = A2 + gp * kUP + cp;
          const int na = Ly.in_dim >> 4;
          if (l == 0) u16p_outer<K, 0, NA0, NPT>(pt, G, na, zl, al);
          else if (l == 1) u16p_outer<K, NA0, NKT, NPT>(pt, G, na, zl, al);
          else u16p_outer<K, NA0 + NKT, NKT, NPT>(pt, G, na, zl, al);
        }
        PINN_STAMP(ST_BWD_STREAM);
        if constexpr (MRG && COEF) {
          if (l == 0 && net.enc == ENC_FOURIER && kon) {
            f32x4 pa[kUPackMax];
#pragma unroll
            for (int j = 0; j < kUPackMax; ++j) pa[j] = f32x4{0.0f, 0.0f, 0.0f, 0.0f};
            u16p_gemm<true>(pa, G, Ly.W, Ly.ld, coff, u16_wload<true>(Ly.W, Ly.ld, coff, 0), u16_wload<true>(Ly.W, Ly.ld, coff, 1),
                            Ly.out_dim >> 4, X + boff);
            const int M = net.enc_out >> 1;
            float part = 0.0f;
#pragma unroll
            for (int j = 0; j < kUPackMax; ++j) {
              if (j < G) {
                const f32x4 val = *reinterpret_cast<const f32x4*>(A2 + eoff + 4 * j * kUP);
#pragma unroll
                for (int r = 0; r < 4; ++r) {
                  const int jf = frowp + r;
                  part = fmaf(pa[j][r], fourier_coef_partial_merged(ep[jf < M ? jf : jf - M], val[r]), part);
                }
              }
            }
            cadd(part, sp == 1);
          }
        }
      }

      if (net.enc == ENC_LINEAR && (net.d_encW || (MRG && COEF))) {
        const int H = net.enc_out;
        const bool enc_sums = !(MRG && COEF) || net.d_encW != nullptr;
        U16_BARRIER(ST_ENC_BWD);
        if (16 * wv < H) {
#pragma unroll
          for (int j = 0; j < kUPackMax; ++j) {
            if (j < G) {
              f32x4 ab[K];
              u16_get<K>(park + eoff + 4 * j * kUP, ab);
#pragma unroll
              for (int r = 0; r < 4; ++r) {
                float z[K], abv[K], zb[K];
                u16_enc_preact<NT, NX>(ep, din, xin, frowp + r, 4 * j + qp, z);
#pragma unroll
                for (int s = 0; s < K; ++s) abv[s] = ab[s][r];
                if constexpr (MRG) cadd(act_bwd_merged<ACT>(net.enc_param, mcoef(), z, abv, zb), sp == 0);
                else act_bwd<ACT, NT, NX>(net.enc_param, z, abv, zb);
#pragma unroll
                for (int s = 0; s < K; ++s) ab[s][r] = zb[s];
              }
              if (enc_sums) u16_put<K>(X + eoff + 4 * j * kUP, ab);
            }
          }
        }
        U16_BARRIER(ST_ENC_BWD);
        if (enc_sums && tp < H) {
          float gb = 0.0f, gt = 0.0f, gx = 0.0f;
          float gw[kMaxDin] = {0.0f, 0.0f, 0.0f, 0.0f};
          for (int n = 0; n < 4 * G; ++n) {
            const float vv = X[n * kUP + tp];
            gb += vv;
#pragma unroll
            for (int cc = 0; cc < kMaxDin; ++cc)
              if (cc < din) gw[cc] = fmaf(vv, xin[cc * kU + n], gw[cc]);
            if constexpr (NT >= 1) gt += X[1 * kUImgS + n * kUP + tp];
            if constexpr (NX >= 1) gx += X[(1 + NT) * kUImgS + n * kUP + tp];
          }
#pragma unroll
          for (int cc = 0; cc < kMaxDin; ++cc) pl[(kPersist + cc) * kUH + tp] += gw[cc] + (cc == din - 1 ? gt : 0.0f) + (cc == 0 ? gx : 0.0f);
          pl[(kPersist + kMaxDin) * kUH + tp] += gb;
        }
        PINN_STAMP(ST_ENC_BWD);
      }
    }
    __syncthreads();
  }
#endif

  const int tf = u16_opaque(tid);
  const int cf = tf & 15, frowf = 16 * wv + 4 * ((tf & 63) >> 4);
  const long long doff = det_row_offset(a);
  if (a.mode == MODE_PDE && a.loss_sum && wv == 0) {
    float sacc = tf < kU ? psl[tf] : 0.0f;
#pragma unroll
    for (int o = 8; o > 0; o >>= 1) sacc += __shfl_xor(sacc, o);
    if (tf == 0) grad_put(a.loss_sum, sacc, doff, a.flush_store != 0);
  }
#ifdef PINN_STAMPS
  auto write_stamps = [&]() {
    if (a.stamps && (tf & 63) == 0) {
      st_acc[ST_TOTAL] = pinn_now() - st_begin;
      for (int i = 0; i < kNumStamps; ++i) a.stamps[((long long)blockIdx.x * kUWaves + wv) * kNumStamps + i] = st_acc[i];
    }
  };
  if constexpr (!BWD) write_stamps();
#endif
  if constexpr (!BWD) return;
  if constexpr (COEF && MRG) {
    float sc = pcl[tf];
#pragma unroll
    for (int o = 32; o > 0; o >>= 1) sc += __shfl_xor(sc, o);
    if ((tf & 63) == 0) UP[wv] = sc;
    __syncthreads();
    if (a.mode == MODE_PDE && a.pde.dcoef && tf == 0) {
      float st = 0.0f;
#pragma unroll
      for (int w = 0; w < kUWaves; ++w) st += UP[w];
      a.pde.dcoef[doff] = -st;
      a.pde.dcoef[doff + 1] = 0.0f;
    }
  } else if constexpr (COEF) {
    if (a.mode == MODE_PDE && a.pde.dcoef && wv == 0) {
      float s0 = tf < kU ? X[tf * kUP + kUH] : 0.0f, s1 = tf < kU ? X[tf * kUP + kUH + 1] : 0.0f;
#pragma unroll
      for (int o = 8; o > 0; o >>= 1) {
        s0 += __shfl_xor(s0, o);
        s1 += __shfl_xor(s1, o);
      }
      if (tf == 0) {
        a.pde.dcoef[doff] = s0;
        a.pde.dcoef[doff + 1] = s1;
      }
    }
  }
  if (net.db_out && wv == 0) {
    float gsum = tf < kU ? psl[kU + tf] : 0.0f;
#pragma unroll
    for (int o = 8; o > 0; o >>= 1) gsum += __shfl_xor(gsum, o);
    if (tf == 0) net.db_out[doff] = gsum;
  }
  if (net.enc == ENC_LINEAR && net.d_encW && tf < net.enc_out) {
#pragma unroll
    for (int cc = 0; cc < kMaxDin; ++cc)
      if (cc < din) net.d_encW[doff + tf * din + cc] = pl[(kPersist + cc) * kUH + tf];
    if (net.d_encb) net.d_encb[doff + tf] = pl[(kPersist + kMaxDin) * kUH + tf];
  }
  const f32x4 pdw = row16_sum4(*reinterpret_cast<const f32x4*>(pdwl + 4 * tf));
  if (net.dw_out && cf == 0 && frowf < net.h_last) *reinterpret_cast<f32x4*>(net.dw_out + doff + frowf) = pdw;
#pragma unroll
  for (int p = 0; p < kPersist; ++p) {
    if (p < nl) {
      const LayerDev Lp = uniform_layer(net.layer[p]);
      if (Lp.db && tf < Lp.out_dim) Lp.db[doff + tf] = pl[p * kUH + tf];
      if (16 * wv >= Lp.out_dim) continue;
      if (Lp.dW) {
        const int na = Lp.in_dim >> 4;
        const int off = p == 0 ? 0 : p == 1 ? NA0 : NA0 + NKT;
        float* base = Lp.dW + doff + (long long)frowf * Lp.ld + cf;
#pragma unroll
        for (int t = 0; t < NPT; ++t) {
          if (t >= off && t - off < na && (p != 0 || t < NA0) && (p != 1 || t < NA0 + NKT)) {
#pragma unroll
            for (int r = 0; r < 4; ++r) base[(long long)r * Lp.ld + 16 * (t - off)] = pt[t][r];
          }
        }
      }
    }
  }
#ifdef PINN_STAMPS
  PINN_STAMP(ST_BWD_FLUSH);
  write_stamps();
#endif
}

struct U16Plan {
  long long rounds;
  long long first_tail;
  int groups;
};
inline U16Plan jet_u16_tail_plan(long long N, int grid, bool packed) {
  U16Plan p;
  const long long per_round = (long long)kU * grid;
  p.rounds = N / per_round;
  p.first_tail = p.rounds * per_round;
  const long long M = N - p.first_tail;
  p.groups = (int)((M + 4LL * grid - 1) / (4LL * grid));
  if (!packed && p.groups > 0) p.groups = 4;
  return p;
}
inline void jet_u16_set_plan(KernelArgs& a, int grid, bool packed) {
  const U16Plan p = jet_u16_tail_plan(a.N, grid, packed);
  const bool pack = p.groups >= 1 && p.groups <= kUPackMax;
  a.u16_loop_points = pack ? p.first_tail : a.N;
  a.u16_tail_groups = pack ? p.groups : 0;
}

inline size_t jet_u16_lds_bytes(int K) {
  return sizeof(float) * ((size_t)4 * K * kUImgS + kUWaves * K * kU + 2 * kMaxDin * kU + (1 + kPersist) * kUH +
                          (kMaxDin + 1) * kUH + (kPersist + kMaxDin + 1) * kUH + 4 * kUThreads + 2 * kU + kMaxDin * kU);
}
constexpr size_t jet_u16m_lds_bytes(bool coef, bool bwd) {
  return sizeof(float) * ((size_t)(bwd ? 5 : 4) * 3 * kUImgS + kUWaves * 3 * kU + 2 * kMaxDin * kU + (1 + kPersist) * kUH +
                          (kMaxDin + 1) * kUH + (kPersist + kMaxDin + 1) * kUH + 4 * kUThreads + 2 * kU + kMaxDin * kU +
                          (coef ? kUThreads : 0));
}
static_assert(jet_u16m_lds_bytes(true, true) <= 160 * 1024 && jet_u16m_lds_bytes(false, true) == 146048 &&
                  jet_u16m_lds_bytes(false, false) == 120704,
              "the merged units' five images and running sums fit the CU's LDS");


inline bool jet_u16_fits(const NetDev& n, int K) {
  if (K > 4 || n.n_layers < 1 || n.n_layers > kPersist || jet_wide_hmax(n.hmax) != 128) return false;
  if (n.layer[0].in_dim > 64) return false;
  for (int l = 0; l < n.n_layers; ++l)
    if (n.layer[l].in_dim % 16 || n.layer[l].out_dim % 16 || n.layer[l].in_dim > kUH || n.layer[l].out_dim > kUH) return false;
  return jet_u16_lds_bytes(K) <= 160 * 1024;
}

template <int ACT, int NT, int NX>
hipError_t launch_jet_u16_act(const KernelArgs& a, bool bwd, int grid, hipStream_t stream) {
  constexpr int K = 1 + NT + NX;
  auto kern = bwd ? jet_kernel_u16<ACT, NT, NX, true, 4> : jet_kernel_u16<ACT, NT, NX, false, 4>;
  hipError_t e = allow_full_lds(reinterpret_cast<const void*>(kern));
  if (e != hipSuccess) return e;
  hipLaunchKernelGGL(kern, dim3(grid), dim3(kUThreads), jet_u16_lds_bytes(K), stream, a);
  return hipGetLastError();
}

template <int ACT, int NT, int NX>
hipError_t launch_jet_u16_coef(const KernelArgs& a, int grid, hipStream_t stream) {
  constexpr int K = 1 + NT + NX;
  auto kern = jet_kernel_u16<ACT, NT, NX, true, 4, true>;
  hipError_t e = allow_full_lds(reinterpret_cast<const void*>(kern));
  if (e != hipSuccess) return e;
  hipLaunchKernelGGL(kern, dim3(grid), dim3(kUThreads), jet_u16_lds_bytes(K), stream, a);
  return hipGetLastError();
}

template <int ACT>
hipError_t launch_jet_u16m_act(const KernelArgs& a, bool bwd, int grid, hipStream_t stream) {
  auto kern = bwd ? jet_kernel_u16<ACT, 1, 1, true, 4, false, true> : jet_kernel_u16<ACT, 1, 1, false, 4, false, true>;
  hipError_t e = allow_full_lds(reinterpret_cast<const void*>(kern));
  if (e != hipSuccess) return e;
  hipLaunchKernelGGL(kern, dim3(grid), dim3(kUThreads), jet_u16m_lds_bytes(false, bwd), stream, a);
  return hipGetLastError();
}
template <int ACT>
hipError_t launch_jet_u16m_coef(const KernelArgs& a, int grid, hipStream_t stream) {
  auto kern = jet_kernel_u16<ACT, 1, 1, true, 4, true, true>;
  hipError_t e = allow_full_lds(reinterpret_cast<const void*>(kern));
  if (e != hipSuccess) return e;
  hipLaunchKernelGGL(kern, dim3(grid), dim3(kUThreads), jet_u16m_lds_bytes(true, true), stream, a);
  return hipGetLastError();
}

}
```

pinns-rl-pde_amd/csrc/pinn_abi.hip:

```cpp
#include <hip/hip_runtime.h>

#include <cstdarg>
#include <cstdio>
#include <cstdlib>
#include <cstring>

#include "jet_kernel_u16.h"
#include "lm_engine.h"

namespace pinn {
#define PINN_DECL(nt, nx) hipError_t launch_jetw_##nt##_##nx(const KernelArgs&, bool, int, hipStream_t);
PINN_DECL(0, 0)
PINN_DECL(1, 0)
PINN_DECL(1, 1)
PINN_DECL(1, 2)
PINN_DECL(1, 3)
PINN_DECL(1, 4)
PINN_DECL(2, 0)
PINN_DECL(2, 2)
#undef PINN_DECL
#define PINN_DECLU1(nt, nx, a) hipError_t launch_jetu_##nt##_##nx##_a##a(const KernelArgs&, bool, int, hipStream_t);
#ifdef PINN_DEV
#define PINN_DECLU(nt, nx) PINN_DECLU1(nt, nx, 0)
#else
#define PINN_DECLU(nt, nx) PINN_DECLU1(nt, nx, 0) PINN_DECLU1(nt, nx, 1) PINN_DECLU1(nt, nx, 2) PINN_DECLU1(nt, nx, 3) PINN_DECLU1(nt, nx, 4)
#endif
PINN_DECLU(0, 0)
PINN_DECLU(1, 0)
PINN_DECLU(1, 1)
PINN_DECLU(1, 2)
PINN_DECLU(2, 0)
#undef PINN_DECLU
#undef PINN_DECLU1
#ifndef PINN_DEV
#define PINN_DECLC1(p, nt, nx, a) hipError_t launch_jet##p##_##nt##_##nx##_a##a(const KernelArgs&, int, hipStream_t);
#define PINN_DECLC(p, nt, nx) PINN_DECLC1(p, nt, nx, 0) PINN_DECLC1(p, nt, nx, 1) PINN_DECLC1(p, nt, nx, 2) PINN_DECLC1(p, nt, nx, 3) PINN_DECLC1(p, nt, nx, 4)
PINN_DECLC(wc, 1, 1)
PINN_DECLC(wc, 1, 2)
PINN_DECLC(wc, 1, 4)
PINN_DECLC(wc, 2, 0)
PINN_DECLC(wc, 2, 2)
PINN_DECLC(uc, 1, 1)
PINN_DECLC(uc, 1, 2)
PINN_DECLC(uc, 2, 0)
#undef PINN_DECLC
#undef PINN_DECLC1
#endif

#if !defined(PINN_DEV)
#define PINN_DECLM(a) hipError_t launch_jetum_a##a(const KernelArgs&, bool, int, hipStream_t); hipError_t launch_jetumc_a##a(const KernelArgs&, int, hipStream_t);
PINN_DECLM(0) PINN_DECLM(1) PINN_DECLM(2) PINN_DECLM(3) PINN_DECLM(4)
#undef PINN_DECLM
#elif defined(PINN_DEV_MERGED)
hipError_t launch_jetum_a0(const KernelArgs&, bool, int, hipStream_t);
#endif

#ifdef PINN_STAMPS
static unsigned long long* g_stamps = nullptr;
#endif

static thread_local char g_err[512] = "";

static int fail(int code, const char* fmt, ...) {
  va_list ap;
  va_start(ap, fmt);
  vsnprintf(g_err, sizeof(g_err), fmt, ap);
  va_end(ap);
  return code;
}
}

extern "C" int pinn_internal_fail(int code, const char* msg) { return pinn::fail(code, "%s", msg); }

namespace pinn {

static int num_cus() {
  static int cached = 0;
  if (cached) return cached;
  int dev = 0, cus = 0;
  if (hipGetDevice(&dev) == hipSuccess &&
      hipDeviceGetAttribute(&cus, hipDeviceAttributeMultiprocessorCount, dev) == hipSuccess && cus > 0) {
    cached = cus;
    return cus;
  }
  (void)hipGetLastError();
  return 256;
}


static bool force_lm() {
  static const bool v = [] {
    const char* e = getenv("PINN_KERNEL");
    return e && !strcmp(e, "lm");
  }();
  return v;
}

static float act_param_of(int act, float user) {
  switch (act) {
    case PINN_ACT_SIN: return user;
    case PINN_ACT_RELU: return 0.0f;
    case PINN_ACT_LEAKY_RELU: return 0.01f;
    case PINN_ACT_IDENTITY: return 1.0f;
    default: return 0.0f;
  }
}

static bool build_wide(const PinnNetDesc* d, const float* const* w, float* const* g, NetDev* out, int* misaligned = nullptr) {
  if (d->arch != PINN_ARCH_FOURIER && d->arch != PINN_ARCH_FEEDFORWARD && d->arch != PINN_ARCH_SIREN) return false;
  if (d->flags & (PINN_FLAG_LAYER_NORM | PINN_FLAG_LAYER_MAJOR)) return false;
  NetDev n;
  memset(&n, 0, sizeof(n));
  n.din = d->input_dim;
  const int act = d->arch == PINN_ARCH_SIREN ? PINN_ACT_SIN : d->activation;
  const float par = act_param_of(act, d->act_param);
  static float sixteen_aligned[4] __attribute__((aligned(16)));
  auto W = [&](int i) -> const float* { return w ? w[i] : sixteen_aligned; };
  auto G = [&](int i) -> float* { return g ? g[i] : nullptr; };
  int first_mfma, wbase;
  if (d->arch == PINN_ARCH_FOURIER) {
    if (d->mapping_size <= 0 || (2 * d->mapping_size) % 8) return false;
    n.enc = ENC_FOURIER;
    n.enc_out = 2 * d->mapping_size;
    n.encW = W(0);
    first_mfma = 0;
    wbase = 1;
  } else {
    n.enc = ENC_LINEAR;
    n.enc_out = d->widths[0];
    n.encW = W(0);
    n.encb = W(1);
    n.d_encW = G(0);
    n.d_encb = G(1);
    n.enc_act = act;
    n.enc_param = par;
    first_mfma = 1;
    wbase = 0;
    if (n.enc_out % 32) return false;
  }
  int prev = n.enc_out, hmax = (n.enc_out + 31) / 32 * 32;
  n.n_layers = 0;
  for (int i = first_mfma; i < d->num_linear - 1; ++i) {
    const int wd = d->widths[i];
    if (wd % 32 || wd <= 0 || wd > 128 || prev % 8) return false;
    LayerDev& L = n.layer[n.n_layers++];
    L.W = W(wbase + 2 * i);
    L.b = W(wbase + 2 * i + 1);
    L.dW = G(wbase + 2 * i);
    L.db = G(wbase + 2 * i + 1);
    L.in_dim = prev;
    L.ld = prev;
    L.out_dim = wd;
    L.act = act;
    L.act_param = par;
    if (reinterpret_cast<uintptr_t>(L.W) & 15) {
      if (misaligned) *misaligned = wbase + 2 * i;
      return false;
    }
    prev = wd;
    if (wd > hmax) hmax = wd;
  }
  const int io = d->num_linear - 1;
  n.w_out = W(wbase + 2 * io);
  n.b_out = W(wbase + 2 * io + 1);
  n.dw_out = G(wbase + 2 * io);
  n.db_out = G(wbase + 2 * io + 1);
  n.h_last = prev;
  if (prev % 32 || hmax > 128) return false;
  n.hmax = hmax;
  *out = n;
  return true;
}

static bool wide_store_flush_on() {
  static const bool v = [] {
    const char* e = getenv("PINN_WIDE_STORE_FLUSH");
    return !(e && atoi(e) == 0);
  }();
  return v;
}

constexpr int kFlushRows = 8;

struct DetTable {
  int n;
  float* user[2 * PINN_MAX_LINEAR + 8];
  unsigned off[2 * PINN_MAX_LINEAR + 8], cnt[2 * PINN_MAX_LINEAR + 8];
  unsigned lead[2 * PINN_MAX_LINEAR + 8];
  unsigned stride;
};

__global__ void wide_det_reduce(const DetTable tab, const float* slab, int rows) {
  const unsigned it = blockIdx.y;
  for (unsigned e = blockIdx.x * blockDim.x + threadIdx.x; e < tab.cnt[it]; e += gridDim.x * blockDim.x) {
    float s = 0.0f;
    for (int b = 0; b < rows; ++b) s += slab[(size_t)b * tab.stride + tab.off[it] + tab.lead[it] + e];
    tab.user[it][e] += s;
  }
}

__global__ __launch_bounds__(256) void wide_rows_reduce(const DetTable tab, const float* slab, int rows) {
  __shared__ float part[8][128];
  const unsigned it = blockIdx.y;
  const unsigned lead = tab.lead[it], end = lead + tab.cnt[it];
  const unsigned cnt4 = (end + 3u) & ~3u;
  const int el = threadIdx.x & 31, rg = threadIdx.x >> 5;
  for (unsigned e0 = blockIdx.x * 128u; e0 < cnt4; e0 += gridDim.x * 128u) {
    const unsigned e = e0 + 4u * el;
    float s0 = 0.0f, s1 = 0.0f, s2 = 0.0f, s3 = 0.0f;
    if (e < cnt4) {
      const float* src = slab + tab.off[it] + e;
#pragma unroll 8
      for (int b = rg; b < rows; b += 8) {
        const float4 v = *reinterpret_cast<const float4*>(src + (size_t)b * tab.stride);
        s0 += v.x; s1 += v.y; s2 += v.z; s3 += v.w;
      }
    }
    part[rg][4 * el + 0] = s0;
    part[rg][4 * el + 1] = s1;
    part[rg][4 * el + 2] = s2;
    part[rg][4 * el + 3] = s3;
    __syncthreads();
    if (threadIdx.x < 128 && e0 + threadIdx.x >= lead && e0 + threadIdx.x < end) {
      float t = 0.0f;
#pragma unroll
      for (int g = 0; g < 8; ++g) t += part[g][threadIdx.x];
      tab.user[it][e0 + threadIdx.x - lead] += t;
    }
    __syncthreads();
  }
}

enum WideFlush { FLUSH_DIRECT = 0, FLUSH_STORE = 1, FLUSH_TWO_LEVEL = 2, FLUSH_DET_SLAB = 3 };

static WideFlush wide_flush(const PinnNetDesc* d, const NetDev& n, int grid, bool bwd) {
  if (bwd && n.n_layers <= kPersist && wide_store_flush_on()) return FLUSH_STORE;
  if (d->flags & PINN_FLAG_DETERMINISTIC) return FLUSH_DET_SLAB;
  if (bwd && grid > kFlushRows) return FLUSH_TWO_LEVEL;
  return FLUSH_DIRECT;
}

static int wide_slab_rows(WideFlush f, int grid) {
  return f == FLUSH_DIRECT ? 0 : f == FLUSH_TWO_LEVEL ? kFlushRows : grid;
}

static float* det_slot(DetTable& t, float* slab, float* user, unsigned count) {
  if (!user) return nullptr;
  const int i = t.n++;
  t.user[i] = user;
  t.off[i] = t.stride;
  t.cnt[i] = count;
  t.stride += (count + 3u) & ~3u;
  return slab + t.off[i];
}

static void det_redirect(NetDev& n, float*& loss_sum, float*& dcoef, float* slab, DetTable& t) {
  memset(&t, 0, sizeof(t));
  static float dummy;
  float* base = slab ? slab : &dummy;
  auto slot = [&](float*& p, unsigned count, bool sizing_always) {
    if (slab) p = det_slot(t, base, p, count);
    else if (p || sizing_always) t.stride += (count + 3u) & ~3u;
  };
  const bool sizing = slab == nullptr;
  if (n.enc == ENC_LINEAR) {
    slot(n.d_encW, (unsigned)(n.enc_out * n.din), sizing);
    slot(n.d_encb, (unsigned)n.enc_out, sizing);
  }
  for (int l = 0; l < n.n_layers; ++l) {
    slot(n.layer[l].dW, (unsigned)(n.layer[l].out_dim * n.layer[l].ld), sizing);
    slot(n.layer[l].db, (unsigned)n.layer[l].out_dim, sizing);
  }
  slot(n.dw_out, (unsigned)n.h_last, sizing);
  slot(n.db_out, 1u, sizing);
  const unsigned loss_off = t.stride;
  slot(loss_sum, 1u, sizing);
  if (slab && dcoef) {
    const int i = t.n++;
    t.user[i] = dcoef;
    t.off[i] = loss_off;
    t.lead[i] = 1;
    t.cnt[i] = 2;
    dcoef = slab + loss_off + 1;
  }
  if (t.stride == 0) t.stride = 4;
}

static int check_orders(int nt, int nx) {
  if (nt < 0 || nt > 2) return fail(PINN_ERR_BAD_ORDER, "Temporal derivative order %d is not supported. Maximum order is 2.", nt);
  if (nx < 0 || nx > 4) return fail(PINN_ERR_BAD_ORDER, "Spatial derivative order %d is not supported. Maximum order is 4.", nx);
  return PINN_OK;
}

static bool stream_set_compiled(int nt, int nx) {
  static const int sets[][2] = {{0, 0}, {1, 0}, {1, 1}, {1, 2}, {1, 3}, {1, 4}, {2, 0}, {2, 2}};
  for (auto& s : sets)
    if (s[0] == nt && s[1] == nx) return true;
  return false;
}

static int space_axis_of(const PinnNetDesc* d) { return (d->flags & PINN_FLAG_SPACE_AXIS_MASK) >> 8; }

static int space_dir_bits(const PinnNetDesc* d) { return d->flags & PINN_FLAG_SPACE_DIRECTION_MASK; }

static bool stream_set_admitted(const PinnNetDesc* d, int nt, int nx) {
  const bool space_only = nt == 0 && nx >= 1 && nx <= 4;
  if (space_dir_bits(d) != 0) {
    char lerr[8];
    return lm::lm_check(d, lerr, sizeof(lerr)) != PINN_OK || space_only;
  }
  if (stream_set_compiled(nt, nx)) return true;
  return space_axis_of(d) != 0 && space_only;
}

static int refuse_axis(const PinnNetDesc* d, const char* entry) {
  if (d && space_axis_of(d) != 0)
    return fail(PINN_ERR_UNSUPPORTED, "%s: PINN_FLAG_SPACE_AXIS(%d) is set, and the compiled PDE kinds differentiate along the first "
                "space axis only (derivatives along further axes: pinn_jet_forward + pinn_term_residual_axes)", entry, space_axis_of(d));
  if (d && space_dir_bits(d) != 0)
    return fail(PINN_ERR_UNSUPPORTED, "%s: PINN_FLAG_SPACE_DIRECTION is set, and the compiled PDE kinds differentiate along the first "
                "space axis only (mixed derivatives: pinn_jet_forward + pinn_term_residual_mixed)", entry);
  return PINN_OK;
}

static hipError_t dispatch_wide(int nt, int nx, const KernelArgs& a, bool bwd, int grid, hipStream_t st) {
#define PINN_CASE2(NT_, NX_) \
  if (nt == NT_ && nx == NX_) return launch_jetw_##NT_##_##NX_(a, bwd, grid, st);
#define PINN_CASE(NT_, NX_) PINN_CASE2(NT_, NX_)
#ifdef PINN_DEV
  PINN_CASE(PINN_DEV_NT, PINN_DEV_NX)
#else
  PINN_CASE(0, 0) PINN_CASE(1, 0) PINN_CASE(1, 1) PINN_CASE(1, 2) PINN_CASE(1, 3) PINN_CASE(1, 4) PINN_CASE(2, 0) PINN_CASE(2, 2)
#endif
#undef PINN_CASE
#undef PINN_CASE2
  return hipErrorInvalidValue;
}

static bool use_wide(const PinnNetDesc* d, const float* const* w, float* const* g, int K, bool bwd, NetDev* n, int* misaligned = nullptr) {
  if (force_lm()) return false;
  if (space_axis_of(d) != 0 || space_dir_bits(d) != 0) return false;
  if (!build_wide(d, w, g, n, misaligned)) return false;
  return jet_wide_fits(K, n->hmax, bwd, n->n_layers);
}

static bool u16_set_compiled(int nt, int nx) {
#ifdef PINN_DEV
  return nt == PINN_DEV_NT && nx == PINN_DEV_NX;
#else
  static const int sets[][2] = {{0, 0}, {1, 0}, {1, 1}, {1, 2}, {2, 0}};
  for (auto& s : sets)
    if (s[0] == nt && s[1] == nx) return true;
  return false;
#endif
}

static bool widec_set_compiled(int nt, int nx) {
#ifdef PINN_DEV
  return false;
#else
  static const int sets[][2] = {{1, 1}, {1, 2}, {1, 4}, {2, 0}, {2, 2}};
  for (auto& s : sets)
    if (s[0] == nt && s[1] == nx) return true;
  return false;
#endif
}
static bool u16c_set_compiled(int nt, int nx) {
#ifdef PINN_DEV
  return false;
#else
  return (nt == 1 && (nx == 1 || nx == 2)) || (nt == 2 && nx == 0);
#endif
}

static bool use_u16(const PinnNetDesc* d, const NetDev& n, int nt, int nx, bool bwd, bool coef = false) {
  (void)bwd;
  if ((d->flags & PINN_FLAG_WIDE_TILE32) || !(coef ? u16c_set_compiled(nt, nx) : u16_set_compiled(nt, nx))) return false;
  if (wide_flush(d, n, 0, true) != FLUSH_STORE || !jet_u16_fits(n, 1 + nt + nx)) return false;
  const int fam = jet_wide_act_family(n);
#ifdef PINN_DEV
  if (fam != PINN_ACT_TANH) return false;
#endif
  char unit[64];
  snprintf(unit, sizeof(unit), coef ? "jet_u16c_%d_%d_%d:" : "jet_u16_%d_%d_%d:", nt, nx, fam);
  return strstr(pinn_build_info(), unit) == nullptr;
}

static bool u16_unit_packed(const NetDev& n, int nt, int nx, bool coef) {
  char unit[64];
  snprintf(unit, sizeof(unit), coef ? "nopack jet_u16c_%d_%d_%d " : "nopack jet_u16_%d_%d_%d ", nt, nx, jet_wide_act_family(n));
  return strstr(pinn_build_info(), unit) == nullptr;
}

static bool use_merged(const PinnNetDesc* d, const NetDev& n, const PinnPdeDesc* pde, int nt, int nx, int mode) {
  if (mode != MODE_PDE || !pde || pde->kind != PINN_PDE_BURGERS || pde->dimension != 1 || nt != 1 || nx != 2) return false;
  if (d->flags & PINN_FLAG_PLAIN_STREAMS) return false;
  const int fam = jet_wide_act_family(n);
#if defined(PINN_DEV) && !defined(PINN_DEV_MERGED)
  return false;
#elif defined(PINN_DEV)
  return fam == PINN_ACT_TANH && use_u16(d, n, nt, nx, true, false);
#else
  if (!use_u16(d, n, nt, nx, true, false) || !use_u16(d, n, nt, nx, true, true)) return false;
  char unit[64];
  snprintf(unit, sizeof(unit), "jet_u16m_%d:", fam);
  if (strstr(pinn_build_info(), unit)) return false;
  snprintf(unit, sizeof(unit), "jet_u16mc_%d:", fam);
  return strstr(pinn_build_info(), unit) == nullptr;
#endif
}

static bool u16m_unit_packed(const NetDev& n, bool coef) {
  char unit[64];
  snprintf(unit, sizeof(unit), coef ? "nopack jet_u16mc_%d " : "nopack jet_u16m_%d ", jet_wide_act_family(n));
  return strstr(pinn_build_info(), unit) == nullptr;
}

static hipError_t dispatch_u16m(bool coef, const KernelArgs& a, bool bwd, int grid, hipStream_t st) {
  [[maybe_unused]] const int fam = jet_wide_act_family(a);
#if !defined(PINN_DEV)
#define PINN_MCASE(A_) \
  if (fam == A_) return coef ? launch_jetumc_a##A_(a, grid, st) : launch_jetum_a##A_(a, bwd, grid, st);
  PINN_MCASE(0) PINN_MCASE(1) PINN_MCASE(2) PINN_MCASE(3) PINN_MCASE(4)
#undef PINN_MCASE
#elif defined(PINN_DEV_MERGED)
  if (!coef && fam == 0) return launch_jetum_a0(a, bwd, grid, st);
#endif
  return hipErrorInvalidValue;
}

static hipError_t dispatch_coef(bool u16, int nt, int nx, const KernelArgs& a, int grid, hipStream_t st) {
#ifndef PINN_DEV
  const int fam = jet_wide_act_family(a);
#define PINN_CCASE1(P_, NT_, NX_, A_) \
  if (nt == NT_ && nx == NX_ && fam == A_) return launch_jet##P_##_##NT_##_##NX_##_a##A_(a, grid, st);
#define PINN_CCASE(P_, NT_, NX_) PINN_CCASE1(P_, NT_, NX_, 0) PINN_CCASE1(P_, NT_, NX_, 1) PINN_CCASE1(P_, NT_, NX_, 2) PINN_CCASE1(P_, NT_, NX_, 3) PINN_CCASE1(P_, NT_, NX_, 4)
  if (u16) {
    PINN_CCASE(uc, 1, 1) PINN_CCASE(uc, 1, 2) PINN_CCASE(uc, 2, 0)
  } else {
    PINN_CCASE(wc, 1, 1) PINN_CCASE(wc, 1, 2) PINN_CCASE(wc, 1, 4) PINN_CCASE(wc, 2, 0) PINN_CCASE(wc, 2, 2)
  }
#undef PINN_CCASE
#undef PINN_CCASE1
#endif
  return hipErrorInvalidValue;
}

static hipError_t dispatch_u16(int nt, int nx, const KernelArgs& a, bool bwd, int grid, hipStream_t st) {
  const int fam = jet_wide_act_family(a);
#define PINN_UCASE1(NT_, NX_, A_) \
  if (nt == NT_ && nx == NX_ && fam == A_) return launch_jetu_##NT_##_##NX_##_a##A_(a, bwd, grid, st);
#ifdef PINN_DEV
#define PINN_UCASE(NT_, NX_) PINN_UCASE1(NT_, NX_, 0)
  PINN_UCASE(PINN_DEV_NT, PINN_DEV_NX)
#else
#define PINN_UCASE(NT_, NX_) PINN_UCASE1(NT_, NX_, 0) PINN_UCASE1(NT_, NX_, 1) PINN_UCASE1(NT_, NX_, 2) PINN_UCASE1(NT_, NX_, 3) PINN_UCASE1(NT_, NX_, 4)
  PINN_UCASE(0, 0) PINN_UCASE(1, 0) PINN_UCASE(1, 1) PINN_UCASE(1, 2) PINN_UCASE(2, 0)
#endif
#undef PINN_UCASE
#undef PINN_UCASE1
  return hipErrorInvalidValue;
}

static size_t wide_tape_floats(const PinnNetDesc* d, const NetDev& n, int nt, int nx, bool bwd, int grid, bool coef = false) {
  if (!bwd || use_u16(d, n, nt, nx, bwd, coef)) return 0;
  return (size_t)jet_tape_floats_per_wg(1 + nt + nx, n.n_layers, 1) * grid;
}

static int wide_grid(const NetDev& n, int K, long long N, bool bwd) {
  (void)n;
  (void)K;
  (void)bwd;
  const long long ntiles = (N + kT - 1) / kT;
  long long g = num_cus();
  if (g > ntiles) g = ntiles;
  return (int)(g < 1 ? 1 : g);
}

static int validate_table(const PinnNetDesc* net, const void* table, int num_tensors, const char* what) {
  if (!net) return fail(PINN_ERR_BAD_DESC, "null descriptor");
  const int want = lm::lm_expected_tensors(net);
  if (want < 0) return fail(PINN_ERR_UNSUPPORTED, "architecture id %d has no kernel", net->arch);
  if (!table) return fail(PINN_ERR_BAD_DESC, "%s table is null", what);
  if (num_tensors != want)
    return fail(PINN_ERR_BAD_DESC, "%s table has %d entries; the state_dict of this architecture has %d", what, num_tensors, want);
  return PINN_OK;
}

static int run(const PinnNetDesc* net, const float* const* weights, float* const* grads, int num_tensors,
               const PinnPdeDesc* pde, const float* x, const float* t, int64_t N, int nt, int nx, int mode,
               float grad_scale, float* const* jets_out, const float* const* jets_bar, float* residual_out,
               float* loss_sum, void* workspace, size_t ws_bytes, bool bwd, void* stream, const float* res_bar = nullptr,
               float* coef_grads = nullptr, float* x_grad = nullptr, float* t_grad = nullptr, bool lm_only = false,
               const float* coef_dev = nullptr) {
  int rc = validate_table(net, weights, num_tensors, "weights");
  if (rc) return rc;
  if (bwd && grads && (rc = validate_table(net, grads, num_tensors, "weight_grads"))) return rc;
  if (N <= 0) return PINN_OK;
  if (!x && net->input_dim > 1) return fail(PINN_ERR_BAD_DESC, "x is null");
  if (!t) return fail(PINN_ERR_BAD_DESC, "t is null");
  if ((rc = check_orders(nt, nx))) return rc;
  if (!stream_set_admitted(net, nt, nx)) return fail(PINN_ERR_UNSUPPORTED, "stream set (nt=%d, nx=%d) is not compiled", nt, nx);
  char lerr[256] = "";
  if ((rc = lm::lm_check(net, lerr, sizeof(lerr)))) return fail(rc, "%s", lerr);
  const int K = 1 + nt + nx;
  PdeDev pd;
  memset(&pd, 0, sizeof(pd));
  if (pde) {
    pd.kind = pde->kind;
    pd.dimension = pde->dimension;
    pd.loss = pde->loss;
    pd.c0 = pde->coef[0];
    pd.c1 = pde->coef[1];
    pd.c2 = pde->coef[2];
    pd.c3 = pde->coef[3];
    pd.huber_delta = pde->huber_delta;
    pd.dcoef = bwd ? coef_grads : nullptr;
    pd.coef_dev = coef_dev;
  }
  const bool inverse = coef_dev != nullptr;
  KernelArgs a;
  memset(&a, 0, sizeof(a));
  int misaligned = -1;
  if (!inverse && coef_grads && !(net->flags & PINN_FLAG_LAYER_MAJOR) && !force_lm() && use_wide(net, nullptr, nullptr, K, bwd, &a.net))
    return fail(PINN_ERR_UNSUPPORTED, "coefficient gradients run on the layer-major engine: set PINN_FLAG_LAYER_MAJOR in the "
                "descriptor for this call and for its pinn_workspace_bytes query");
  bool wide = !lm_only && use_wide(net, weights, grads, K, bwd, &a.net, &misaligned);
  if (!wide && misaligned >= 0)
    return fail(PINN_ERR_MISALIGNED, "weight tensor %d is not 16-byte aligned: the fused kernel of this descriptor reads hidden-layer "
                "weights with 16-byte loads (pass aligned tensors, or set PINN_FLAG_LAYER_MAJOR to take the packing engine)", misaligned);
  if (inverse && !widec_set_compiled(nt, nx)) wide = false;
  if (wide) {
    const int grid = wide_grid(a.net, K, N, bwd);
    a.pde = pd;
    a.x = x;
    a.t = t;
    a.N = N;
    a.mode = mode;
    a.grad_scale = grad_scale;
    for (int s = 0; s < K; ++s) {
      a.jets_out[s] = jets_out ? jets_out[s] : nullptr;
      a.jets_bar[s] = jets_bar ? jets_bar[s] : nullptr;
    }
    a.residual_out = residual_out;
    a.loss_sum = loss_sum;
    a.res_bar = res_bar;
#ifdef PINN_STAMPS
    a.stamps = g_stamps;
#endif
    const WideFlush flush = wide_flush(net, a.net, grid, bwd);
    const bool store_flush = flush == FLUSH_STORE;
    const bool two_level = flush == FLUSH_TWO_LEVEL;
    const bool det = flush != FLUSH_DIRECT;
    const int slab_rows = wide_slab_rows(flush, grid);
    const bool u16 = use_u16(net, a.net, nt, nx, bwd, inverse);
    const size_t tape_floats = wide_tape_floats(net, a.net, nt, nx, bwd, grid, inverse);
    size_t need = tape_floats * sizeof(float);
    DetTable dt;
    dt.n = 0;
    if (det) {
      NetDev probe = a.net;
      float* lprobe = a.loss_sum;
      float* cprobe = a.pde.dcoef;
      det_redirect(probe, lprobe, cprobe, nullptr, dt);
      need += (size_t)dt.stride * slab_rows * sizeof(float);
    }
    if (need > 0 && (!workspace || ws_bytes < need))
      return fail(PINN_ERR_WORKSPACE, "workspace too small: need %zu bytes, got %zu", need, ws_bytes);
    if (need > 0 && (reinterpret_cast<uintptr_t>(workspace) & 15)) return fail(PINN_ERR_MISALIGNED, "workspace is not 16-byte aligned");
    if (tape_floats > 0) {
      a.tape_stride = jet_tape_floats_per_wg(K, a.net.n_layers, 1);
      a.tape = static_cast<float*>(workspace);
    }
    float* slab = nullptr;
    if (det) {
      const unsigned stride = dt.stride;
      slab = static_cast<float*>(workspace) + tape_floats;
      det_redirect(a.net, a.loss_sum, a.pde.dcoef, slab, dt);
      dt.stride = stride;
      a.det_stride = two_level ? -(long long)stride : (long long)stride;
      a.det_mask = slab_rows - 1;
      a.flush_store = store_flush ? 1 : 0;
      if (!store_flush) {
        const hipError_t em = hipMemsetAsync(slab, 0, (size_t)stride * slab_rows * sizeof(float), static_cast<hipStream_t>(stream));
        if (em != hipSuccess) return fail(PINN_ERR_HIP, "HIP error %d: %s", (int)em, hipGetErrorString(em));
      }
    }
    const bool merged = u16 && use_merged(net, a.net, pde, nt, nx, mode);
    if (u16) jet_u16_set_plan(a, grid, merged ? u16m_unit_packed(a.net, inverse) : u16_unit_packed(a.net, nt, nx, inverse));
    hipError_t e = merged  ? dispatch_u16m(inverse, a, bwd, grid, static_cast<hipStream_t>(stream))
                   : inverse ? dispatch_coef(u16, nt, nx, a, grid, static_cast<hipStream_t>(stream))
                   : u16   ? dispatch_u16(nt, nx, a, bwd, grid, static_cast<hipStream_t>(stream))
                           : dispatch_wide(nt, nx, a, bwd, grid, static_cast<hipStream_t>(stream));
    if (e != hipSuccess) return fail(PINN_ERR_HIP, "HIP error %d: %s", (int)e, hipGetErrorString(e));
    if (det && dt.n > 0 && store_flush) {
      hipLaunchKernelGGL(wide_rows_reduce, dim3(136, dt.n), dim3(256), 0, static_cast<hipStream_t>(stream), dt, slab, slab_rows);
      e = hipGetLastError();
      if (e != hipSuccess) return fail(PINN_ERR_HIP, "HIP error %d: %s", (int)e, hipGetErrorString(e));
    } else if (det && dt.n > 0) {
      hipLaunchKernelGGL(wide_det_reduce, dim3(32, dt.n), dim3(256), 0, static_cast<hipStream_t>(stream), dt, slab, slab_rows);
      e = hipGetLastError();
      if (e != hipSuccess) return fail(PINN_ERR_HIP, "HIP error %d: %s", (int)e, hipGetErrorString(e));
    }
    return PINN_OK;
  }
  lm::CallArgs c;
  memset(&c, 0, sizeof(c));
  c.net = net;
  c.weights = weights;
  c.grads = grads;
  c.num_tensors = num_tensors;
  c.pde = pd;
  c.x = x;
  c.t = t;
  c.N = N;
  c.nt = nt;
  c.nx = nx;
  c.mode = mode;
  c.grad_scale = grad_scale;
  c.jets_out = jets_out;
  c.jets_bar = jets_bar;
  c.residual_out = residual_out;
  c.loss_sum = loss_sum;
  c.res_bar = res_bar;
  c.workspace = workspace;
  c.ws_bytes = ws_bytes;
  c.bwd = bwd;
  c.deterministic = (net->flags & PINN_FLAG_DETERMINISTIC) != 0;
  c.stream = static_cast<hipStream_t>(stream);
  c.x_grad = x_grad;
  c.t_grad = t_grad;
  rc = lm::lm_run(c, lerr, sizeof(lerr));
  if (rc) return fail(rc, "%s", lerr);
  return PINN_OK;
}

}

using namespace pinn;

extern "C" {

int pinn_abi_version(void) { return PINN_ABI_VERSION; }

const char* pinn_last_error(void) { return g_err; }

int pinn_num_tensors(const PinnNetDesc* net) {
  if (!net) return fail(PINN_ERR_BAD_DESC, "null descriptor");
  const int n = lm::lm_expected_tensors(net);
  if (n < 0) return fail(PINN_ERR_UNSUPPORTED, "architecture id %d has no kernel", net->arch);
  char lerr[256] = "";
  const int rc = lm::lm_check(net, lerr, sizeof(lerr));
  if (rc) return fail(rc, "%s", lerr);
  return n;
}

int pinn_pde_streams(const PinnPdeDesc* pde, int32_t* time_order, int32_t* space_order) {
  if (!pde || !time_order || !space_order) return fail(PINN_ERR_BAD_DESC, "null argument");
  int nt = 1, nx = 0;
  if (pde->dimension > 1 && pde->kind == PINN_PDE_CONVECTION)
    return fail(PINN_ERR_UNSUPPORTED, "convection with dimension %d: the reference's residual raises for dimension > 1", pde->dimension);
  if (pde->dimension > 1) {
    nt = (pde->kind == PINN_PDE_WAVE || pde->kind == PINN_PDE_PENDULUM) ? 2 : 1;
  } else {
    switch (pde->kind) {
      case PINN_PDE_BURGERS: case PINN_PDE_ALLEN_CAHN: case PINN_PDE_BLACK_SCHOLES: case PINN_PDE_HEAT_LAPLACIAN: nt = 1; nx = 2; break;
      case PINN_PDE_HEAT: case PINN_PDE_CONVECTION: nt = 1; nx = 1; break;
      case PINN_PDE_KDV: nt = 1; nx = 3; break;
      case PINN_PDE_CAHN_HILLIARD: nt = 1; nx = 4; break;
      case PINN_PDE_WAVE: nt = 2; nx = 2; break;
      case PINN_PDE_PENDULUM: nt = 2; nx = 0; break;
      default: return fail(PINN_ERR_BAD_DESC, "unknown pde kind %d", pde->kind);
    }
  }
  *time_order = nt;
  *space_order = nx;
  return PINN_OK;
}

size_t pinn_workspace_bytes(const PinnNetDesc* net, int64_t N, int32_t time_order, int32_t space_order, int32_t backward) {
  if (!net || N <= 0) return 0;
  if (time_order < 0 || time_order > 2 || space_order < 0 || space_order > 4) return 0;
  char lerr[64];
  if (lm::lm_check(net, lerr, sizeof(lerr)) != PINN_OK) return 0;
  const int K = 1 + time_order + space_order;
  const bool bwd = backward != 0;
  NetDev n;
  if (backward != 2 && use_wide(net, nullptr, nullptr, K, bwd, &n)) {
    const int grid = wide_grid(n, K, N, bwd);
    size_t bytes = bwd ? (size_t)jet_tape_floats_per_wg(K, n.n_layers, 1) * sizeof(float) * grid : 0;
    const int rows = wide_slab_rows(wide_flush(net, n, grid, bwd), grid);
    if (rows > 0) {
      DetTable dt;
      float* lprobe = nullptr;
      float* cprobe = nullptr;
      det_redirect(n, lprobe, cprobe, nullptr, dt);
      bytes += (size_t)dt.stride * rows * sizeof(float);
    }
    return bytes;
  }
  return lm::lm_workspace_bytes(net, N, time_order, space_order, bwd, (net->flags & PINN_FLAG_DETERMINISTIC) != 0);
}

int pinn_kernel_for(const PinnNetDesc* net, int64_t N, int32_t time_order, int32_t space_order, int32_t backward,
                    PinnKernelInfo* out) {
  if (!net || !out) return fail(PINN_ERR_BAD_DESC, "null argument");
  if (N <= 0) return fail(PINN_ERR_BAD_DESC, "N = %lld: a call on no points launches nothing", (long long)N);
  if (backward < 0 || backward > 2) return fail(PINN_ERR_BAD_DESC, "backward = %d: 0, 1 or 2", backward);
  int rc = check_orders(time_order, space_order);
  if (rc) return rc;
  if (!stream_set_admitted(net, time_order, space_order))
    return fail(PINN_ERR_UNSUPPORTED, "stream set (nt=%d, nx=%d) is not compiled", time_order, space_order);
  char lerr[256] = "";
  if ((rc = lm::lm_check(net, lerr, sizeof(lerr)))) return fail(rc, "%s", lerr);
  PinnKernelInfo r;
  memset(&r, 0, sizeof(r));
  r.time_order = time_order;
  r.space_order = space_order;
  r.backward = backward;
  r.act_family = r.hmax = r.na0 = r.grid = r.flush = -1;
  const int K = 1 + time_order + space_order;
  const bool bwd = backward != 0;
  NetDev n;
  if (backward != 2 && use_wide(net, nullptr, nullptr, K, bwd, &n)) {
    r.engine = 1;
    r.act_family = jet_wide_act_family(n);
    jet_wide_variant(n, bwd, &r.hmax, &r.na0);
    r.grid = wide_grid(n, K, N, bwd);
    r.flush = wide_flush(net, n, r.grid, bwd);
    char unit[64];
    snprintf(unit, sizeof(unit), "jet_wide_%d_%d_%d:", time_order, space_order, r.act_family);
    r.default_mfma_form = strstr(pinn_build_info(), unit) != nullptr;
  }
  *out = r;
  return PINN_OK;
}

int pinn_lm_plan(const PinnNetDesc* net, int64_t N, int32_t time_order, int32_t space_order, int32_t backward,
                 PinnLmNodePlan* out, int32_t max_records) {
  PinnKernelInfo r;
  int rc = pinn_kernel_for(net, N, time_order, space_order, backward, &r);
  if (rc) return rc;
  char lerr[256] = "";
  rc = lm::lm_plan(net, time_order, space_order, backward, out, max_records, lerr, sizeof(lerr));
  if (rc < 0) return fail(rc, "%s", lerr);
  return rc;
}

int pinn_kernel_name(const PinnNetDesc* net, int64_t N, int32_t time_order, int32_t space_order, int32_t backward,
                     char* buf, size_t len) {
  if (!buf || len == 0) return fail(PINN_ERR_BAD_DESC, "null or empty name buffer");
  PinnKernelInfo r;
  const int rc = pinn_kernel_for(net, N, time_order, space_order, backward, &r);
  if (rc) return rc;
  const char* name = "layer_major";
  if (r.engine == 1) {
    NetDev n;
    build_wide(net, nullptr, nullptr, &n);
    name = use_u16(net, n, time_order, space_order, backward == 1) ? "jet_kernel_u16" : "jet_kernel_wide";
  }
  snprintf(buf, len, "%s", name);
  return PINN_OK;
}

int pinn_unit_tail_plan(int64_t N, int32_t grid, int64_t* rounds, int32_t* groups, int64_t* first_tail_point) {
  if (N < 0 || grid < 1) return fail(PINN_ERR_BAD_DESC, "pinn_unit_tail_plan: N = %lld, grid = %d", (long long)N, (int)grid);
  const U16Plan p = jet_u16_tail_plan(N, grid, true);
  if (rounds) *rounds = p.rounds;
  if (groups) *groups = p.groups;
  if (first_tail_point) *first_tail_point = p.first_tail;
  return PINN_OK;
}

int pinn_jet_forward(const PinnNetDesc* net, const float* const* weights, int32_t num_tensors, const float* x,
                     const float* t, int64_t N, int32_t time_order, int32_t space_order, float* const* jets_out,
                     void* workspace, size_t ws_bytes, void* stream) {
  if (!jets_out) return fail(PINN_ERR_BAD_DESC, "jets_out is null");
  return run(net, weights, nullptr, num_tensors, nullptr, x, t, N, time_order, space_order, MODE_JETS, 0.0f, jets_out,
             nullptr, nullptr, nullptr, workspace, ws_bytes, false, stream);
}

int pinn_jet_backward(const PinnNetDesc* net, const float* const* weights, int32_t num_tensors, const float* x,
                      const float* t, int64_t N, int32_t time_order, int32_t space_order,
                      const float* const* jet_cotangents, float* const* weight_grads, void* workspace, size_t ws_bytes,
                      void* stream) {
  if (!jet_cotangents || !weight_grads) return fail(PINN_ERR_BAD_DESC, "null cotangents or weight_grads");
  return run(net, weights, weight_grads, num_tensors, nullptr, x, t, N, time_order, space_order, MODE_JETS, 0.0f, nullptr,
             jet_cotangents, nullptr, nullptr, workspace, ws_bytes, true, stream);
}

int pinn_jet_backward_inputs(const PinnNetDesc* net, const float* const* weights, int32_t num_tensors, const float* x,
                             const float* t, int64_t N, int32_t time_order, int32_t space_order,
                             const float* const* jet_cotangents, float* const* weight_grads, float* x_grad, float* t_grad,
                             void* workspace, size_t ws_bytes, void* stream) {
  if (!jet_cotangents) return fail(PINN_ERR_BAD_DESC, "null cotangents");
  if (net && weight_grads) {
    const int rc = validate_table(net, weight_grads, num_tensors, "weight_grads");
    if (rc) return rc;
  }
  if (net && net->input_dim <= 1) x_grad = nullptr;
  if (!weight_grads && !x_grad && !t_grad) {
    int rc = validate_table(net, weights, num_tensors, "weights");
    if (rc || N <= 0) return rc;
    if ((rc = check_orders(time_order, space_order))) return rc;
    if (!stream_set_admitted(net, time_order, space_order))
      return fail(PINN_ERR_UNSUPPORTED, "stream set (nt=%d, nx=%d) is not compiled", time_order, space_order);
    char lerr[256] = "";
    if ((rc = lm::lm_check(net, lerr, sizeof(lerr)))) return fail(rc, "%s", lerr);
    return PINN_OK;
  }
  return run(net, weights, weight_grads, num_tensors, nullptr, x, t, N, time_order, space_order, MODE_JETS, 0.0f, nullptr,
             jet_cotangents, nullptr, nullptr, workspace, ws_bytes, true, stream, nullptr, nullptr, x_grad, t_grad, true);
}

int pinn_residual_forward(const PinnNetDesc* net, const float* const* weights, int32_t num_tensors,
                          const PinnPdeDesc* pde, const float* x, const float* t, int64_t N, float* residual_out,
                          float* loss_sum_out, void* workspace, size_t ws_bytes, void* stream) {
  int32_t nt, nx;
  int rc = refuse_axis(net, "pinn_residual_forward");
  if (rc) return rc;
  rc = pinn_pde_streams(pde, &nt, &nx);
  if (rc) return rc;
  return run(net, weights, nullptr, num_tensors, pde, x, t, N, nt, nx, MODE_PDE, 0.0f, nullptr, nullptr, residual_out,
             loss_sum_out, workspace, ws_bytes, false, stream);
}

int pinn_residual_loss_grad(const PinnNetDesc* net, const float* const* weights, int32_t num_tensors,
                            const PinnPdeDesc* pde, const float* x, const float* t, int64_t N, float grad_scale,
                            float* residual_out, float* loss_sum_out, float* const* weight_grads, void* workspace,
                            size_t ws_bytes, void* stream) {
  if (!weight_grads) return fail(PINN_ERR_BAD_DESC, "weight_grads is null");
  int32_t nt, nx;
  int rc = refuse_axis(net, "pinn_residual_loss_grad");
  if (rc) return rc;
  rc = pinn_pde_streams(pde, &nt, &nx);
  if (rc) return rc;
  return run(net, weights, weight_grads, num_tensors, pde, x, t, N, nt, nx, MODE_PDE, grad_scale, nullptr, nullptr,
             residual_out, loss_sum_out, workspace, ws_bytes, true, stream);
}

int pinn_residual_loss_grad_coef(const PinnNetDesc* net, const float* const* weights, int32_t num_tensors,
                                 const PinnPdeDesc* pde, const float* x, const float* t, int64_t N, float grad_scale,
                                 float* residual_out, float* loss_sum_out, float* const* weight_grads, float* coef_grads,
                                 void* workspace, size_t ws_bytes, void* stream) {
  if (!weight_grads) return fail(PINN_ERR_BAD_DESC, "weight_grads is null");
  int32_t nt, nx;
  int rc = refuse_axis(net, "pinn_residual_loss_grad_coef");
  if (rc) return rc;
  rc = pinn_pde_streams(pde, &nt, &nx);
  if (rc) return rc;
  return run(net, weights, weight_grads, num_tensors, pde, x, t, N, nt, nx, MODE_PDE, grad_scale, nullptr, nullptr,
             residual_out, loss_sum_out, workspace, ws_bytes, true, stream, nullptr, coef_grads);
}

static int inverse_route(const PinnNetDesc* net, int nt, int nx, NetDev* n) {
  if (!widec_set_compiled(nt, nx) || !use_wide(net, nullptr, nullptr, 1 + nt + nx, true, n)) return 0;
  return use_u16(net, *n, nt, nx, true, true) ? 2 : 1;
}

static int inverse_query(const PinnNetDesc* net, const PinnPdeDesc* pde, int64_t N, int32_t* nt, int32_t* nx) {
  if (!net || !pde) return fail(PINN_ERR_BAD_DESC, "null descriptor");
  if (N <= 0) return fail(PINN_ERR_BAD_DESC, "N = %lld: a call on no points launches nothing", (long long)N);
  int rc = refuse_axis(net, "pinn_residual_loss_grad_inverse");
  if (rc) return rc;
  rc = pinn_pde_streams(pde, nt, nx);
  if (rc) return rc;
  if (!stream_set_compiled(*nt, *nx)) return fail(PINN_ERR_UNSUPPORTED, "stream set (nt=%d, nx=%d) is not compiled", *nt, *nx);
  char lerr[256] = "";
  if ((rc = lm::lm_check(net, lerr, sizeof(lerr)))) return fail(rc, "%s", lerr);
  return PINN_OK;
}

int pinn_residual_loss_grad_inverse(const PinnNetDesc* net, const float* const* weights, int32_t num_tensors,
                                    const PinnPdeDesc* pde, const float* coef_values, const float* x, const float* t,
                                    int64_t N, float grad_scale, float* residual_out, float* loss_sum_out,
                                    float* const* weight_grads, float* coef_grads, void* workspace, size_t ws_bytes,
                                    void* stream) {
  if (!weight_grads) return fail(PINN_ERR_BAD_DESC, "weight_grads is null");
  if (!coef_values) return fail(PINN_ERR_BAD_DESC, "coef_values is null: the coefficients of this call live on the device");
  int32_t nt, nx;
  int rc = refuse_axis(net, "pinn_residual_loss_grad_inverse");
  if (rc) return rc;
  rc = pinn_pde_streams(pde, &nt, &nx);
  if (rc) return rc;
  PinnPdeDesc p = *pde;
  p.coef[0] = p.coef[1] = p.coef[2] = p.coef[3] = 0.0f;
  return run(net, weights, weight_grads, num_tensors, &p, x, t, N, nt, nx, MODE_PDE, grad_scale, nullptr, nullptr,
             residual_out, loss_sum_out, workspace, ws_bytes, true, stream, nullptr, coef_grads, nullptr, nullptr, false,
             coef_values);
}

size_t pinn_inverse_workspace_bytes(const PinnNetDesc* net, const PinnPdeDesc* pde, int64_t N) {
  int32_t nt, nx;
  if (inverse_query(net, pde, N, &nt, &nx) != PINN_OK) return 0;
  NetDev n;
  if (inverse_route(net, nt, nx, &n) == 0)
    return lm::lm_workspace_bytes(net, N, nt, nx, true, (net->flags & PINN_FLAG_DETERMINISTIC) != 0);
  const int K = 1 + nt + nx;
  const int grid = wide_grid(n, K, N, true);
  size_t bytes = (size_t)jet_tape_floats_per_wg(K, n.n_layers, 1) * sizeof(float) * grid;
  const int rows = wide_slab_rows(wide_flush(net, n, grid, true), grid);
  if (rows > 0) {
    DetTable dt;
    float* lprobe = nullptr;
    float* cprobe = nullptr;
    det_redirect(n, lprobe, cprobe, nullptr, dt);
    bytes += (size_t)dt.stride * rows * sizeof(float);
  }
  return bytes;
}

int pinn_inverse_kernel_name(const PinnNetDesc* net, const PinnPdeDesc* pde, int64_t N, char* buf, size_t len) {
  if (!buf || len == 0) return fail(PINN_ERR_BAD_DESC, "null or empty name buffer");
  int32_t nt, nx;
  const int rc = inverse_query(net, pde, N, &nt, &nx);
  if (rc) return rc;
  NetDev n;
  const int route = inverse_route(net, nt, nx, &n);
  snprintf(buf, len, "%s", route == 2 ? "jet_kernel_u16" : route == 1 ? "jet_kernel_wide" : "layer_major");
  return PINN_OK;
}

int pinn_residual_backward(const PinnNetDesc* net, const float* const* weights, int32_t num_tensors,
                           const PinnPdeDesc* pde, const float* x, const float* t, int64_t N,
                           const float* residual_cotangent, float* const* weight_grads, void* workspace,
                           size_t ws_bytes, void* stream) {
  if (!weight_grads || !residual_cotangent) return fail(PINN_ERR_BAD_DESC, "null cotangent or weight_grads");
  int32_t nt, nx;
  int rc = refuse_axis(net, "pinn_residual_backward");
  if (rc) return rc;
  rc = pinn_pde_streams(pde, &nt, &nx);
  if (rc) return rc;
  return run(net, weights, weight_grads, num_tensors, pde, x, t, N, nt, nx, MODE_PDE, 0.0f, nullptr, nullptr, nullptr,
             nullptr, workspace, ws_bytes, true, stream, residual_cotangent);
}

#ifdef PINN_STAMPS
void pinn_debug_set_stamps(void* device_buffer) { g_stamps = static_cast<unsigned long long*>(device_buffer); }
#endif

}
```

Measured before the change: 136.5 million.

## Add fixed-shape specialization of merged u16 jet kernel for 2-64-128x3 Fourier nets

```diff
diff --git a/include/pinn_jet.h b/include/pinn_jet.h
--- a/include/pinn_jet.h
+++ b/include/pinn_jet.h
@@ -17,6 +17,7 @@
 #define PINN_FLAG_LAYER_MAJOR 4
 #define PINN_FLAG_WIDE_TILE32 8
 #define PINN_FLAG_PLAIN_STREAMS 16
+#define PINN_FLAG_GENERIC_UNITS 32
 #define PINN_FLAG_SPACE_AXIS(a) ((a) << 8)
 #define PINN_FLAG_SPACE_AXIS_MASK 0x300
 #define PINN_FLAG_SPACE_DIRECTION(d0, d1, d2) \
@@ -170,6 +171,7 @@
                                     void* stream);
 size_t pinn_inverse_workspace_bytes(const PinnNetDesc* net, const PinnPdeDesc* pde, int64_t N);
 int pinn_inverse_kernel_name(const PinnNetDesc* net, const PinnPdeDesc* pde, int64_t N, char* buf, size_t len);
+int pinn_residual_unit_name(const PinnNetDesc* net, const PinnPdeDesc* pde, int64_t N, char* buf, size_t len);
 
 int pinn_residual_backward(const PinnNetDesc* net, const float* const* weights, int32_t num_tensors,
                            const PinnPdeDesc* pde, const float* x, const float* t, int64_t N,
diff --git a/pinns-rl-pde_amd/_lib.py b/pinns-rl-pde_amd/_lib.py
--- a/pinns-rl-pde_amd/_lib.py
+++ b/pinns-rl-pde_amd/_lib.py
@@ -18,6 +18,7 @@
 PINN_FLAG_LAYER_MAJOR = 4
 PINN_FLAG_WIDE_TILE32 = 8
 PINN_FLAG_PLAIN_STREAMS = 16
+PINN_FLAG_GENERIC_UNITS = 32
 PINN_FLAG_SPACE_AXIS_MASK = 0x300
 
 
@@ -79,7 +80,7 @@
     "pinn_inverse_workspace_bytes", "pinn_inverse_kernel_name", "pinn_adaptive_adam_step", "pinn_lbfgs_state_bytes",
     "pinn_lbfgs_scratch_bytes", "pinn_lbfgs_direction", "pinn_lbfgs_eval_stats", "pinn_fd_stencil_points", "pinn_fd_smoothness",
     "pinn_unit_tail_plan", "pinn_term_residual", "pinn_causal_weights", "pinn_term_residual_axes",
-    "pinn_term_residual_mixed", "pinn_lm_plan", "pinn_term_residual_system",
+    "pinn_term_residual_mixed", "pinn_lm_plan", "pinn_term_residual_system", "pinn_residual_unit_name",
 )
 
 
@@ -237,6 +238,8 @@
         lib.pinn_inverse_workspace_bytes.argtypes = [P(PinnNetDesc), P(PinnPdeDesc), i64]
         lib.pinn_inverse_kernel_name.restype = ctypes.c_int
         lib.pinn_inverse_kernel_name.argtypes = [P(PinnNetDesc), P(PinnPdeDesc), i64, ctypes.c_char_p, sz]
+        lib.pinn_residual_unit_name.restype = ctypes.c_int
+        lib.pinn_residual_unit_name.argtypes = [P(PinnNetDesc), P(PinnPdeDesc), i64, ctypes.c_char_p, sz]
         lib.pinn_point_losses.restype = ctypes.c_int
         lib.pinn_point_losses.argtypes = [vp, i32, i32, P(i32), P(i32), P(vp), P(f32), i32, f32, vp, vp, vp, f32, f32, i32, vp, vp]
         lib.pinn_jet_losses.restype = ctypes.c_int
@@ -306,6 +309,12 @@
     return buf.value.decode("ascii")
 
 
+def residual_unit_name(prog, pd, N: int) -> str:
+    buf = ctypes.create_string_buffer(64)
+    check(load().pinn_residual_unit_name(ctypes.byref(prog.desc), ctypes.byref(pd), int(N), buf, len(buf)))
+    return buf.value.decode("ascii")
+
+
 def u16_tail_plan(N: int, grid: int) -> tuple:
     r, g, f = ctypes.c_int64(), ctypes.c_int32(), ctypes.c_int64()
     check(load().pinn_unit_tail_plan(int(N), int(grid), ctypes.byref(r), ctypes.byref(g), ctypes.byref(f)))
diff --git a/pinns-rl-pde_amd/csrc/jet_kernel_u16.h b/pinns-rl-pde_amd/csrc/jet_kernel_u16.h
--- a/pinns-rl-pde_amd/csrc/jet_kernel_u16.h
+++ b/pinns-rl-pde_amd/csrc/jet_kernel_u16.h
@@ -17,6 +17,11 @@
 constexpr int kUH = 128;
 constexpr int kUImgS = kU * kUP;
 
+struct U16FixedShape {
+  int din, enc_out, layers, in0, width;
+};
+constexpr U16FixedShape kUFixed = {2, 64, 3, 64, 128};
+
 __device__ __forceinline__ f32x4 mfma16(float a, float b, f32x4 c) {
   return __builtin_amdgcn_mfma_f32_16x16x4f32(a, b, c, 0, 0, 0);
 }
@@ -44,14 +49,14 @@
   if constexpr (NX >= 1) z[1 + NT] = ep[j];
 }
 
-template <int ACT, int NT, int NX, bool MRG = false>
+template <int ACT, int NT, int NX, bool MRG = false, bool FIXED = false>
 __device__ __forceinline__ void u16_encode(const NetDev& net, const float* ep, const float* xin, float* dst, int tid, float cc = 0.0f) {
   constexpr int K = 1 + NT + NX;
   const int n = tid & 15;
-  const int din = net.din;
+  const int din = FIXED ? kUFixed.din : net.din;
   float* row = dst + n * kUP;
-  if (net.enc == ENC_FOURIER) {
-    const int M = net.enc_out >> 1;
+  if (FIXED || net.enc == ENC_FOURIER) {
+    const int M = FIXED ? kUFixed.enc_out >> 1 : net.enc_out >> 1;
 #pragma unroll 1
     for (int m = tid >> 4; m < M; m += kUThreads / kU) {
       float z[K], ys[K], yc[K];
@@ -355,9 +360,33 @@
   return v;
 }
 
-template <int ACT, int NT, int NX, bool BWD, int NA0, bool COEF = false, bool MRG = false>
+struct U16FixedLayers {
+  const float *W0, *W1, *W2;
+  float ap0, ap1, ap2;
+};
+__device__ __forceinline__ LayerDev u16_fixed_layer(const U16FixedLayers f, int l, bool scalar_sizes = false) {
+  LayerDev u = {};
+  u.W = l == 0 ? f.W0 : l == 1 ? f.W1 : f.W2;
+  int in_dim = l == 0 ? kUFixed.in0 : kUFixed.width, out_dim = kUFixed.width;
+  if (scalar_sizes) asm("" : "+s"(in_dim), "+s"(out_dim));
+  u.in_dim = in_dim;
+  u.out_dim = out_dim;
+  int ld = u.in_dim;
+  asm("" : "+s"(ld));
+  u.ld = ld;
+  u.act_param = l == 0 ? f.ap0 : l == 1 ? f.ap1 : f.ap2;
+  return u;
+}
+#define U16_LAYER(l) (FIXED ? u16_fixed_layer(fix, (l)) : uniform_layer(net.layer[(l)]))
+#define U16_LAYER_P(l) (FIXED ? u16_fixed_layer(fix, (l), true) : uniform_layer(net.layer[(l)]))
+#define U16_HAS_DW(l, Ly) (FIXED ? ((fnull >> (l)) & 1u) == 0u : (Ly).dW != nullptr)
+#define U16_HAS_DB(l, Ly) (FIXED ? ((fnull >> (4 + (l))) & 1u) == 0u : (Ly).db != nullptr)
+#define U16_LAYER_UNROLL FIXED ? kPersist : 1
+
+template <int ACT, int NT, int NX, bool BWD, int NA0, bool COEF = false, bool MRG = false, bool FIXED = false>
 __global__ __launch_bounds__(kUThreads, 1) void jet_kernel_u16(const KernelArgs a) {
   static_assert(!MRG || (NT == 1 && NX == 1), "the merged set is laid out as the (1,1) set");
+  static_assert(!FIXED || (MRG && NA0 == kUFixed.in0 / 16), "the fixed shape is a merged unit's");
   constexpr int K = 1 + NT + NX;
   constexpr int NKT = kUH / 16;
   constexpr int NPT = NA0 + (kPersist - 1) * NKT;
@@ -394,8 +423,8 @@
   const int wv = __builtin_amdgcn_readfirstlane(tid >> 6);
   const int lane = tid & 63;
   const int g = lane >> 4, c = lane & 15;
-  const int din = net.din;
-  const int nl = net.n_layers;
+  const int din = FIXED ? kUFixed.din : net.din;
+  const int nl = FIXED ? kUFixed.layers : net.n_layers;
 #if PINN_U16_PACK
   const long long NL = a.u16_loop_points;
 #else
@@ -532,6 +561,25 @@
   fetch_coords(blockIdx.x);
   put_coords(xin2, blockIdx.x);
   if constexpr (MRG) fetch_coords(blockIdx.x + gridDim.x);
+  [[maybe_unused]] U16FixedLayers fix = {};
+  [[maybe_unused]] unsigned fnull = 0u;
+  if constexpr (FIXED) {
+    auto resident_w = [&](int l) -> const float* {
+      unsigned long long wp = reinterpret_cast<unsigned long long>(net.layer[l].W);
+      asm("" : "+s"(wp));
+      using gfloat = const float __attribute__((address_space(1)));
+      return (const float*)(gfloat*)wp;
+    };
+    auto resident_ap = [&](int l) -> float {
+      unsigned ap = __float_as_uint(net.layer[l].act_param);
+      asm("" : "+s"(ap));
+      return __uint_as_float(ap);
+    };
+    fix = {resident_w(0), resident_w(1), resident_w(2), resident_ap(0), resident_ap(1), resident_ap(2)};
+#pragma unroll
+    for (int l = 0; l < kPersist; ++l) fnull |= (net.layer[l].dW ? 0u : 1u << l) | (net.layer[l].db ? 0u : 16u << l);
+    asm("" : "+s"(fnull));
+  }
   int xpar = 0;
 
   for (long long u = blockIdx.x; u < nunits; u += gridDim.x) {
@@ -543,7 +591,7 @@
     if constexpr (!MRG) fetch_coords(u + gridDim.x);
     f32x4 w0, w1;
     {
-      const LayerDev L0 = uniform_layer(net.layer[0]);
+      const LayerDev L0 = U16_LAYER(0);
       const unsigned off = u16_rows_off(16 * wv < L0.out_dim ? 16 * wv : 0, L0.ld, c, g);
       w0 = u16_wload<false>(L0.W, L0.ld, off, 0);
       w1 = u16_wload<false>(L0.W, L0.ld, off, L0.in_dim > 16 ? 1 : 0);
@@ -551,13 +599,14 @@
     PINN_STAMP(ST_STAGE);
     float* src = (MRG || (nl & 1)) ? X : A2;
     float* dst = (MRG || (nl & 1)) ? A2 : X;
-    u16_encode<ACT, NT, NX, MRG>(net, ep, xin, src, u16_opaque(tid), mcoef());
+    u16_encode<ACT, NT, NX, MRG, FIXED>(net, ep, xin, src, u16_opaque(tid), mcoef());
     U16_BARRIER(ST_ENCODE);
 
     f32x4 acc[K];
+#pragma unroll U16_LAYER_UNROLL
     for (int l = 0; l < nl; ++l) {
-      const LayerDev Ly = uniform_layer(net.layer[l]);
-      const bool on = 16 * wv < Ly.out_dim;
+      const LayerDev Ly = U16_LAYER(l);
+      const bool on = FIXED || 16 * wv < Ly.out_dim;
       const bool last = l + 1 == nl;
 #pragma unroll
       for (int s = 0; s < K; ++s) acc[s] = f32x4{0.0f, 0.0f, 0.0f, 0.0f};
@@ -574,7 +623,7 @@
       PINN_STAMP(ST_FWD_GEMM);
       if (!last) {
         {
-          const LayerDev Ln = uniform_layer(net.layer[l + 1]);
+          const LayerDev Ln = U16_LAYER(l + 1);
           const unsigned off = u16_rows_off(16 * wv < Ln.out_dim ? 16 * wv : 0, Ln.ld, c, g);
           w0 = u16_wload<false>(Ln.W, Ln.ld, off, 0);
           w1 = u16_wload<false>(Ln.W, Ln.ld, off, Ln.in_dim > 16 ? 1 : 0);
@@ -626,7 +675,7 @@
         for (int w = 0; w < kUWaves; ++w) v += UP[(w * K + s) * kU + c];
         j[s] = v;
       }
-      if (a.mode == MODE_JETS) {
+      if (!FIXED && a.mode == MODE_JETS) {
 #pragma unroll
         for (int s = 0; s < K; ++s) {
           if (writer && ok && a.jets_out[s]) a.jets_out[s][p] = j[s];
@@ -669,7 +718,7 @@
     if (tid < kU) psl[kU + c] += ub[0];
     f32x4 ab[K];
     {
-      const LayerDev Lz = uniform_layer(net.layer[nl - 1]);
+      const LayerDev Lz = U16_LAYER(nl - 1);
       const f32x4 w4 = *reinterpret_cast<const f32x4*>(wb + frow);
 #pragma unroll
       for (int s = 0; s < K; ++s) ab[s] = w4 * ub[s];
@@ -701,10 +750,11 @@
     }
     PINN_STAMP(ST_B0);
 
+#pragma unroll U16_LAYER_UNROLL
     for (int l = nl - 1; l >= 0; --l) {
-      const LayerDev Ly = uniform_layer(net.layer[l]);
-      const bool on = 16 * wv < Ly.out_dim;
-      const bool need_abar = l > 0 || net.enc == ENC_LINEAR;
+      const LayerDev Ly = U16_LAYER(l);
+      const bool on = FIXED || 16 * wv < Ly.out_dim;
+      const bool need_abar = l > 0 || (!FIXED && net.enc == ENC_LINEAR);
       const bool kon = 16 * wv < Ly.in_dim;
       if constexpr (!KEEP) {
         if (l + 1 < nl || nl == 1) U16_BARRIER(ST_BWD_EW);
@@ -714,9 +764,9 @@
       const float* const AP = !KEEP || (l & 1) ? A2 : X;
       float pw = 0.0f;
       if constexpr (KEEP) {
-        if (l > 0) pw = uniform_layer(net.layer[l - 1]).act_param;
+        if (l > 0) pw = U16_LAYER(l - 1).act_param;
       } else if (l > 0) {
-        const LayerDev P = uniform_layer(net.layer[l - 1]);
+        const LayerDev P = U16_LAYER(l - 1);
         pw = P.act_param;
         if (kon) {
           f32x4 rec[K], y[K];
@@ -733,7 +783,7 @@
           u16_put<K>(A2 + ioff, y);
         }
       } else {
-        u16_encode<ACT, NT, NX, MRG>(net, ep, xin, A2, u16_opaque(tid), mcoef());
+        u16_encode<ACT, NT, NX, MRG, FIXED>(net, ep, xin, A2, u16_opaque(tid), mcoef());
       }
       const unsigned coff = u16_cols_off(kon ? 16 * wv : 0, Ly.ld, c, g);
       if (need_abar) {
@@ -741,7 +791,7 @@
         w1 = u16_wload<true>(Ly.W, Ly.ld, coff, 1);
       }
       U16_BARRIER(ST_BWD_PUT);
-      if (Ly.db && tid < Ly.out_dim) {
+      if (U16_HAS_DB(l, Ly) && tid < Ly.out_dim) {
         float gsum = 0.0f;
 #pragma unroll
         for (int n = 0; n < kU; ++n) gsum += ZB[n * kUP + tid];
@@ -751,7 +801,7 @@
       const bool dw_first = wv >= 4;
 #pragma unroll
       for (int half = 0; half < 2; ++half) {
-        if ((half == 0) == dw_first && on && Ly.dW) {
+        if ((half == 0) == dw_first && on && U16_HAS_DW(l, Ly)) {
           const float* zl = ZB + 4 * g * kUP + 16 * wv + c;
           const float* al = AP + 4 * g * kUP + c;
           const int na = Ly.in_dim >> 4;
@@ -777,12 +827,12 @@
       }
       if constexpr (KEEP) {
         if (l == 1 && nl > 2) {
-          u16_encode<ACT, NT, NX, MRG>(net, ep, xin, X, u16_opaque(tid), mcoef());
+          u16_encode<ACT, NT, NX, MRG, FIXED>(net, ep, xin, X, u16_opaque(tid), mcoef());
           PINN_STAMP(ST_ENCODE);
         }
       }
       if constexpr (MRG && COEF) {
-        if (l == 0 && net.enc == ENC_FOURIER && kon) {
+        if (l == 0 && (FIXED || net.enc == ENC_FOURIER) && kon) {
           f32x4 aw[1] = {f32x4{0.0f, 0.0f, 0.0f, 0.0f}};
           {
             const float* xl = ZB + kUImgS + c * kUP + 4 * g;
@@ -795,7 +845,7 @@
               for (int m = 0; m < 4; ++m) aw[0] = mfma16(w[m], xv[m], aw[0]);
             }
           }
-          const int M = net.enc_out >> 1;
+          const int M = FIXED ? kUFixed.enc_out >> 1 : net.enc_out >> 1;
           const f32x4 val = *reinterpret_cast<const f32x4*>(AP + ioff);
           float part = 0.0f;
 #pragma unroll
@@ -808,7 +858,7 @@
       }
     }
 
-    if (net.enc == ENC_LINEAR && (net.d_encW || (MRG && COEF))) {
+    if (!FIXED && net.enc == ENC_LINEAR && (net.d_encW || (MRG && COEF))) {
       const int H = net.enc_out;
       const bool enc_sums = !(MRG && COEF) || net.d_encW != nullptr;
       U16_BARRIER(ST_ENC_BWD);
@@ -873,7 +923,7 @@
     const float* xin = xint;
     f32x4 w0, w1;
     {
-      const LayerDev L0 = uniform_layer(net.layer[0]);
+      const LayerDev L0 = U16_LAYER_P(0);
       const unsigned off = u16_rows_off(16 * wv < L0.out_dim ? 16 * wv : 0, L0.ld, cp, gp);
       w0 = u16_wload<false>(L0.W, L0.ld, off, 0);
       w1 = u16_wload<false>(L0.W, L0.ld, off, L0.in_dim > 16 ? 1 : 0);
@@ -881,11 +931,12 @@
     PINN_STAMP(ST_STAGE);
     float* src = (nl & 1) ? X : A2;
     float* dst = (nl & 1) ? A2 : X;
-    u16_encode<ACT, NT, NX, MRG>(net, ep, xin, src, tp, mcoef());
+    u16_encode<ACT, NT, NX, MRG, FIXED>(net, ep, xin, src, tp, mcoef());
     U16_BARRIER(ST_ENCODE);
 
+#pragma unroll 1
     for (int l = 0; l < nl; ++l) {
-      const LayerDev Ly = uniform_layer(net.layer[l]);
+      const LayerDev Ly = U16_LAYER_P(l);
       const bool on = 16 * wv < Ly.out_dim;
       const bool last = l + 1 == nl;
       f32x4 pa[kUPackMax];
@@ -894,7 +945,7 @@
       if (on) u16p_gemm<false>(pa, G, Ly.W, Ly.ld, u16_rows_off(16 * wv, Ly.ld, cp, gp), w0, w1, Ly.in_dim >> 4, src + boff);
       PINN_STAMP(ST_FWD_GEMM);
       if (!last) {
-        const LayerDev Ln = uniform_layer(net.layer[l + 1]);
+        const LayerDev Ln = U16_LAYER_P(l + 1);
         const unsigned off = u16_rows_off(16 * wv < Ln.out_dim ? 16 * wv : 0, Ln.ld, cp, gp);
         w0 = u16_wload<false>(Ln.W, Ln.ld, off, 0);
         w1 = u16_wload<false>(Ln.W, Ln.ld, off, Ln.in_dim > 16 ? 1 : 0);
@@ -964,7 +1015,7 @@
           for (int w = 0; w < kUWaves; ++w) v += UP[(w * K + s) * kU + pp];
           j[s] = v;
         }
-        if (a.mode == MODE_JETS) {
+        if (!FIXED && a.mode == MODE_JETS) {
 #pragma unroll
           for (int s = 0; s < K; ++s) {
             if (writer && ok && a.jets_out[s]) a.jets_out[s][p] = j[s];
@@ -1006,7 +1057,7 @@
       if (writer) psl[kU + pp] += ub[0];
       f32x4 ab[K];
       {
-        const LayerDev Lz = uniform_layer(net.layer[nl - 1]);
+        const LayerDev Lz = U16_LAYER_P(nl - 1);
         const f32x4 w4 = *reinterpret_cast<const f32x4*>(wb + frowp);
 #pragma unroll
         for (int s = 0; s < K; ++s) ab[s] = w4 * ub[s];
@@ -1038,10 +1089,11 @@
     }
 
     if constexpr (BWD) {
+#pragma unroll 1
       for (int l = nl - 1; l >= 0; --l) {
-        const LayerDev Ly = uniform_layer(net.layer[l]);
+        const LayerDev Ly = U16_LAYER_P(l);
         const bool on = 16 * wv < Ly.out_dim;
-        const bool need_abar = l > 0 || net.enc == ENC_LINEAR;
+        const bool need_abar = l > 0 || (!FIXED && net.enc == ENC_LINEAR);
         const bool kon = 16 * wv < Ly.in_dim;
         auto unpark = [&]() {
 #pragma unroll
@@ -1060,7 +1112,7 @@
         float pw = 0.0f;
         u16_wave_sync();
         if (l > 0) {
-          const LayerDev P = uniform_layer(net.layer[l - 1]);
+          const LayerDev P = U16_LAYER_P(l - 1);
           pw = P.act_param;
           if (kon) {
 #pragma unroll
@@ -1082,7 +1134,7 @@
             }
           }
         } else {
-          u16_encode<ACT, NT, NX, MRG>(net, ep, xin, A2, tp, mcoef());
+          u16_encode<ACT, NT, NX, MRG, FIXED>(net, ep, xin, A2, tp, mcoef());
         }
         const unsigned coff = u16_cols_off(kon ? 16 * wv : 0, Ly.ld, cp, gp);
         if (need_abar) {
@@ -1090,7 +1142,7 @@
           w1 = u16_wload<true>(Ly.W, Ly.ld, coff, 1);
         }
         U16_BARRIER(ST_BWD_PUT);
-        if (Ly.db && tp < Ly.out_dim) {
+        if (U16_HAS_DB(l, Ly) && tp < Ly.out_dim) {
           float gsum = 0.0f;
           for (int n = 0; n < 4 * G; ++n) gsum += X[n * kUP + tp];
           pl[l * kUH + tp] += gsum;
@@ -1126,7 +1178,7 @@
           park = xch;
           PINN_STAMP(ST_BWD_EW);
         }
-        if (on && Ly.dW) {
+        if (on && U16_HAS_DW(l, Ly)) {
           const float* zl = X + gp * kUP + 16 * wv + cp;
           const float* al = A2 + gp * kUP + cp;
           const int na = Ly.in_dim >> 4;
@@ -1136,13 +1188,13 @@
         }
         PINN_STAMP(ST_BWD_STREAM);
         if constexpr (MRG && COEF) {
-          if (l == 0 && net.enc == ENC_FOURIER && kon) {
+          if (l == 0 && (FIXED || net.enc == ENC_FOURIER) && kon) {
             f32x4 pa[kUPackMax];
 #pragma unroll
             for (int j = 0; j < kUPackMax; ++j) pa[j] = f32x4{0.0f, 0.0f, 0.0f, 0.0f};
             u16p_gemm<true>(pa, G, Ly.W, Ly.ld, coff, u16_wload<true>(Ly.W, Ly.ld, coff, 0), u16_wload<true>(Ly.W, Ly.ld, coff, 1),
                             Ly.out_dim >> 4, X + boff);
-            const int M = net.enc_out >> 1;
+            const int M = FIXED ? kUFixed.enc_out >> 1 : net.enc_out >> 1;
             float part = 0.0f;
 #pragma unroll
             for (int j = 0; j < kUPackMax; ++j) {
@@ -1160,7 +1212,7 @@
         }
       }
 
-      if (net.enc == ENC_LINEAR && (net.d_encW || (MRG && COEF))) {
+      if (!FIXED && net.enc == ENC_LINEAR && (net.d_encW || (MRG && COEF))) {
         const int H = net.enc_out;
         const bool enc_sums = !(MRG && COEF) || net.d_encW != nullptr;
         U16_BARRIER(ST_ENC_BWD);
@@ -1261,7 +1313,7 @@
     for (int o = 8; o > 0; o >>= 1) gsum += __shfl_xor(gsum, o);
     if (tf == 0) net.db_out[doff] = gsum;
   }
-  if (net.enc == ENC_LINEAR && net.d_encW && tf < net.enc_out) {
+  if (!FIXED && net.enc == ENC_LINEAR && net.d_encW && tf < net.enc_out) {
 #pragma unroll
     for (int cc = 0; cc < kMaxDin; ++cc)
       if (cc < din) net.d_encW[doff + tf * din + cc] = pl[(kPersist + cc) * kUH + tf];
@@ -1272,7 +1324,11 @@
 #pragma unroll
   for (int p = 0; p < kPersist; ++p) {
     if (p < nl) {
-      const LayerDev Lp = uniform_layer(net.layer[p]);
+      LayerDev Lp = U16_LAYER(p);
+      if constexpr (FIXED) {
+        Lp.dW = uniform_ptr(net.layer[p].dW);
+        Lp.db = uniform_ptr(net.layer[p].db);
+      }
       if (Lp.db && tf < Lp.out_dim) Lp.db[doff + tf] = pl[p * kUH + tf];
       if (16 * wv >= Lp.out_dim) continue;
       if (Lp.dW) {
@@ -1294,6 +1350,12 @@
   write_stamps();
 #endif
 }
+
+#undef U16_LAYER
+#undef U16_LAYER_P
+#undef U16_HAS_DW
+#undef U16_HAS_DB
+#undef U16_LAYER_UNROLL
 
 struct U16Plan {
   long long rounds;
@@ -1359,17 +1421,27 @@
   return hipGetLastError();
 }
 
-template <int ACT>
+inline bool jet_u16_fixed_shape(const NetDev& n) {
+  if (n.enc != ENC_FOURIER || n.din != kUFixed.din || n.enc_out != kUFixed.enc_out || n.n_layers != kUFixed.layers) return false;
+  if (n.h_last != kUFixed.width) return false;
+  for (int l = 0; l < kUFixed.layers; ++l) {
+    const int in = l == 0 ? kUFixed.in0 : kUFixed.width;
+    if (n.layer[l].in_dim != in || n.layer[l].out_dim != kUFixed.width || n.layer[l].ld != in) return false;
+  }
+  return true;
+}
+
+template <int ACT, bool FIXED = false>
 hipError_t launch_jet_u16m_act(const KernelArgs& a, bool bwd, int grid, hipStream_t stream) {
-  auto kern = bwd ? jet_kernel_u16<ACT, 1, 1, true, 4, false, true> : jet_kernel_u16<ACT, 1, 1, false, 4, false, true>;
+  auto kern = bwd ? jet_kernel_u16<ACT, 1, 1, true, 4, false, true, FIXED> : jet_kernel_u16<ACT, 1, 1, false, 4, false, true, FIXED>;
   hipError_t e = allow_full_lds(reinterpret_cast<const void*>(kern));
   if (e != hipSuccess) return e;
   hipLaunchKernelGGL(kern, dim3(grid), dim3(kUThreads), jet_u16m_lds_bytes(false, bwd), stream, a);
   return hipGetLastError();
 }
-template <int ACT>
+template <int ACT, bool FIXED = false>
 hipError_t launch_jet_u16m_coef(const KernelArgs& a, int grid, hipStream_t stream) {
-  auto kern = jet_kernel_u16<ACT, 1, 1, true, 4, true, true>;
+  auto kern = jet_kernel_u16<ACT, 1, 1, true, 4, true, true, FIXED>;
   hipError_t e = allow_full_lds(reinterpret_cast<const void*>(kern));
   if (e != hipSuccess) return e;
   hipLaunchKernelGGL(kern, dim3(grid), dim3(kUThreads), jet_u16m_lds_bytes(true, true), stream, a);
diff --git a/pinns-rl-pde_amd/csrc/jet_u16mf_inst.hip b/pinns-rl-pde_amd/csrc/jet_u16mf_inst.hip
--- /dev/null
+++ b/pinns-rl-pde_amd/csrc/jet_u16mf_inst.hip
@@ -0,0 +1,14 @@
+#include "jet_kernel_u16.h"
+
+#if !defined(PINN_WIDE_ACT)
+#error "compile with -DPINN_WIDE_ACT=<0..4>"
+#endif
+
+#define PINN_CAT2(a, b) a##b
+#define PINN_CATM(a, b) PINN_CAT2(a, b)
+
+namespace pinn {
+hipError_t PINN_CATM(launch_jetumf_a, PINN_WIDE_ACT)(const KernelArgs& a, bool bwd, int grid, hipStream_t stream) {
+  return launch_jet_u16m_act<PINN_WIDE_ACT, true>(a, bwd, grid, stream);
+}
+}
diff --git a/pinns-rl-pde_amd/csrc/jet_u16mfc_inst.hip b/pinns-rl-pde_amd/csrc/jet_u16mfc_inst.hip
--- /dev/null
+++ b/pinns-rl-pde_amd/csrc/jet_u16mfc_inst.hip
@@ -0,0 +1,14 @@
+#include "jet_kernel_u16.h"
+
+#if !defined(PINN_WIDE_ACT)
+#error "compile with -DPINN_WIDE_ACT=<0..4>"
+#endif
+
+#define PINN_CAT2(a, b) a##b
+#define PINN_CATM(a, b) PINN_CAT2(a, b)
+
+namespace pinn {
+hipError_t PINN_CATM(launch_jetumfc_a, PINN_WIDE_ACT)(const KernelArgs& a, int grid, hipStream_t stream) {
+  return launch_jet_u16m_coef<PINN_WIDE_ACT, true>(a, grid, stream);
+}
+}
diff --git a/pinns-rl-pde_amd/csrc/pinn_abi.hip b/pinns-rl-pde_amd/csrc/pinn_abi.hip
--- a/pinns-rl-pde_amd/csrc/pinn_abi.hip
+++ b/pinns-rl-pde_amd/csrc/pinn_abi.hip
@@ -49,10 +49,14 @@
 
 #if !defined(PINN_DEV)
 #define PINN_DECLM(a) hipError_t launch_jetum_a##a(const KernelArgs&, bool, int, hipStream_t); hipError_t launch_jetumc_a##a(const KernelArgs&, int, hipStream_t);
+#define PINN_DECLF(a) hipError_t launch_jetumf_a##a(const KernelArgs&, bool, int, hipStream_t); hipError_t launch_jetumfc_a##a(const KernelArgs&, int, hipStream_t);
 PINN_DECLM(0) PINN_DECLM(1) PINN_DECLM(2) PINN_DECLM(3) PINN_DECLM(4)
+PINN_DECLF(0) PINN_DECLF(2) PINN_DECLF(4)
 #undef PINN_DECLM
+#undef PINN_DECLF
 #elif defined(PINN_DEV_MERGED)
 hipError_t launch_jetum_a0(const KernelArgs&, bool, int, hipStream_t);
+hipError_t launch_jetumf_a0(const KernelArgs&, bool, int, hipStream_t);
 #endif
 
 #ifdef PINN_STAMPS
@@ -416,15 +420,39 @@
   return strstr(pinn_build_info(), unit) == nullptr;
 }
 
-static hipError_t dispatch_u16m(bool coef, const KernelArgs& a, bool bwd, int grid, hipStream_t st) {
+static bool use_fixed_shape(const PinnNetDesc* d, const NetDev& n, bool merged) {
+  if (!merged || (d->flags & PINN_FLAG_GENERIC_UNITS) || !jet_u16_fixed_shape(n)) return false;
+  const int fam = jet_wide_act_family(n);
+  if (fam == PINN_ACT_SIN || fam == PINN_ACT_SIGMOID) return false;
+  const char* info = pinn_build_info();
+  char unit[64];
+#if defined(PINN_DEV)
+  const int forms = 1;
+#else
+  const int forms = 2;
+#endif
+  for (int coef = 0; coef < forms; ++coef) {
+    snprintf(unit, sizeof(unit), coef ? "jet_u16mfc_%d:" : "jet_u16mf_%d:", fam);
+    if (strstr(info, unit)) return false;
+    snprintf(unit, sizeof(unit), coef ? "nopack jet_u16mfc_%d " : "nopack jet_u16mf_%d ", fam);
+    if ((strstr(info, unit) == nullptr) != u16m_unit_packed(n, coef != 0)) return false;
+  }
+  return true;
+}
+
+static hipError_t dispatch_u16m(bool coef, bool fixed, const KernelArgs& a, bool bwd, int grid, hipStream_t st) {
   [[maybe_unused]] const int fam = jet_wide_act_family(a);
 #if !defined(PINN_DEV)
+#define PINN_FCASE(A_) \
+  if (fam == A_ && fixed) return coef ? launch_jetumfc_a##A_(a, grid, st) : launch_jetumf_a##A_(a, bwd, grid, st);
 #define PINN_MCASE(A_) \
   if (fam == A_) return coef ? launch_jetumc_a##A_(a, grid, st) : launch_jetum_a##A_(a, bwd, grid, st);
+  PINN_FCASE(0) PINN_FCASE(2) PINN_FCASE(4)
   PINN_MCASE(0) PINN_MCASE(1) PINN_MCASE(2) PINN_MCASE(3) PINN_MCASE(4)
 #undef PINN_MCASE
+#undef PINN_FCASE
 #elif defined(PINN_DEV_MERGED)
-  if (!coef && fam == 0) return launch_jetum_a0(a, bwd, grid, st);
+  if (!coef && fam == 0) return fixed ? launch_jetumf_a0(a, bwd, grid, st) : launch_jetum_a0(a, bwd, grid, st);
 #endif
   return hipErrorInvalidValue;
 }
@@ -588,7 +616,8 @@
     }
     const bool merged = u16 && use_merged(net, a.net, pde, nt, nx, mode);
     if (u16) jet_u16_set_plan(a, grid, merged ? u16m_unit_packed(a.net, inverse) : u16_unit_packed(a.net, nt, nx, inverse));
-    hipError_t e = merged  ? dispatch_u16m(inverse, a, bwd, grid, static_cast<hipStream_t>(stream))
+    const bool fixed = use_fixed_shape(net, a.net, merged);
+    hipError_t e = merged  ? dispatch_u16m(inverse, fixed, a, bwd, grid, static_cast<hipStream_t>(stream))
                    : inverse ? dispatch_coef(u16, nt, nx, a, grid, static_cast<hipStream_t>(stream))
                    : u16   ? dispatch_u16(nt, nx, a, bwd, grid, static_cast<hipStream_t>(stream))
                            : dispatch_wide(nt, nx, a, bwd, grid, static_cast<hipStream_t>(stream));
@@ -763,6 +792,22 @@
   return PINN_OK;
 }
 
+int pinn_residual_unit_name(const PinnNetDesc* net, const PinnPdeDesc* pde, int64_t N, char* buf, size_t len) {
+  int32_t nt, nx;
+  int rc = pinn_pde_streams(pde, &nt, &nx);
+  if (rc) return rc;
+  rc = pinn_kernel_name(net, N, nt, nx, 1, buf, len);
+  if (rc || strcmp(buf, "jet_kernel_u16") != 0) return rc;
+  NetDev n;
+  build_wide(net, nullptr, nullptr, &n);
+  const int fam = jet_wide_act_family(n);
+  const bool merged = use_merged(net, n, pde, nt, nx, MODE_PDE);
+  if (use_fixed_shape(net, n, merged)) snprintf(buf, len, "jet_u16mf_%d", fam);
+  else if (merged) snprintf(buf, len, "jet_u16m_%d", fam);
+  else snprintf(buf, len, "jet_u16_%d_%d_%d", (int)nt, (int)nx, fam);
+  return PINN_OK;
+}
+
 int pinn_unit_tail_plan(int64_t N, int32_t grid, int64_t* rounds, int32_t* groups, int64_t* first_tail_point) {
   if (N < 0 || grid < 1) return fail(PINN_ERR_BAD_DESC, "pinn_unit_tail_plan: N = %lld, grid = %d", (long long)N, (int)grid);
   const U16Plan p = jet_u16_tail_plan(N, grid, true);
```

Result: faster. 145.0 million (median of 6 runs) (+6.2%).
